# timspilak/cloud_merger

Hardware: NVIDIA B200
Metric: merged+voxel-filtered Mpoints/s (higher is better)
Workload: dtype f32

## Files before the change

### cloud_merger_b200/csrc/cm_api.cu

```cuda
#include <cuda_runtime.h>
#include <dlfcn.h>
#include <sched.h>
#include <nccl.h>

#include <algorithm>
#include <chrono>
#include <cmath>
#include <cstdarg>
#include <cstddef>
#include <cstdio>
#include <cstdlib>
#include <cstring>
#include <limits>
#include <memory>
#include <mutex>
#include <new>
#include <random>
#include <string>
#include <type_traits>
#include <unordered_map>
#include <vector>

#include "../../include/cloud_merger_gpu.h"
#include "cm_kernels.h"
// ... 157 lines not shown
    DevPtr<uint32_t> out_src;
    HostPtr<uint32_t> report;
    cudaStream_t stream = nullptr;
    bool ran = false;
    int64_t launches = 0;
    ZoneParams last{};
    int n_zones_run = 0;
    bool ror_run = false;
  } zw;
  DevPtr<uint32_t> cell_table;
  size_t cell_table_cap = 0;
  DevPtr<float4> stage;
  size_t stage_cap = 0;
  struct SorWs {
    size_t cap = 0;
    DevPtr<float4> sorted_pts;
    DevPtr<float> dist;
    DevPtr<SorStats> stats;
    HostPtr<SorStats> stats_host;
    Event ev[3];
    cudaStream_t stream = nullptr;
    bool ran = false, profiled = false;
    int n_clouds = 0;
    int64_t n_points = 0;
    uint32_t n_valid[CM_MAX_ZONES] = {};
    uint32_t too_few = 0;
  } sw;
  struct PlaneWs {
    size_t cap_draws = 0;
    DevPtr<int32_t> samples_dev;
    DevPtr<int32_t> counts_dev;
    DevPtr<float4> models_dev;
    DevPtr<float> acc_dev;
    HostPtr<int32_t> samples_pin;
    HostPtr<int32_t> counts_pin;
    HostPtr<float4> models_pin;
    HostPtr<float> acc_pin;
  } pw;
  struct ProceedWs {
    size_t cap = 0;
    DevPtr<float4> low, high, rest, planes;
    DevPtr<float4> no_ground, ground;
  } prz;
  std::vector<Slot> slots;
  std::vector<Stream> sensor_stream;
  size_t slot_stride = 0;
  int fill = 0;
  int64_t ticket_counter = 0;
  bool use_graph = true;
  int submit_policy = CM_SUBMIT_LATEST_WINS;
};

namespace {

int fail(cm_handle_t h, int code, const char* fmt, ...) {
  char buf[512];
  va_list ap;
  va_start(ap, fmt);
  vsnprintf(buf, sizeof(buf), fmt, ap);
  va_end(ap);
  if (h) h->last_error = buf;
  return code;
}

#define CM_CUDA(h, expr)                                                                              \
  do {                                                                                                \
    cudaError_t e__ = (expr);                                                                         \
    if (e__ != cudaSuccess) return fail(h, CM_E_CUDA, "%s: %s (%s:%d)", #expr, cudaGetErrorString(e__), \
                                        __FILE__, __LINE__);                                          \
  } while (0)

int numa_node_of_current_device() {
  int dev = 0;
  char bus[64] = {0};
  if (cudaGetDevice(&dev) != cudaSuccess || cudaDeviceGetPCIBusId(bus, (int)sizeof(bus), dev) != cudaSuccess) { cudaGetLastError(); return -1; }
  for (char* c = bus; *c; ++c) *c = (char)tolower(*c);
  char path[160];
  snprintf(path, sizeof(path), "/sys/bus/pci/devices/%s/numa_node", bus);
  FILE* f = fopen(path, "r");
  if (!f) return -1;
  int node = -1;
  if (fscanf(f, "%d", &node) != 1) node = -1;
  fclose(f);
  return node;
}
bool cpus_of_node(int node, cpu_set_t* set) {
  char path[96];
  snprintf(path, sizeof(path), "/sys/devices/system/node/node%d/cpulist", node);
  FILE* f = fopen(path, "r");
  if (!f) return false;
  CPU_ZERO(set);
  int a = 0, b = 0, n = 0;
  char sep = 0;
  while (fscanf(f, "%d", &a) == 1) {
    b = a;
    int c = fgetc(f);
    if (c == '-') { if (fscanf(f, "%d", &b) != 1) break; c = fgetc(f); }
    for (int k = a; k <= b && k < CPU_SETSIZE; ++k) { CPU_SET(k, set); ++n; }
    sep = (char)c;
    if (sep != ',') break;
  }
  fclose(f);
  return n > 0;
}
template <typename T>
cudaError_t pinned_alloc(HostPtr<T>& p, size_t bytes, unsigned flags) {
  static const bool no_numa = getenv("CM_NO_NUMA") != nullptr;
  cpu_set_t old_set, local;
  bool moved = false;
  if (!no_numa) {
    const int node = numa_node_of_current_device();
    if (node >= 0 && cpus_of_node(node, &local) && sched_getaffinity(0, sizeof(old_set), &old_set) == 0) {
      cpu_set_t both;
      CPU_AND(&both, &local, &old_set);
      if (CPU_COUNT(&both) > 0 && !CPU_EQUAL(&both, &old_set)) moved = sched_setaffinity(0, sizeof(both), &both) == 0;
    }
  }
  void* raw = nullptr;
  const cudaError_t e = cudaHostAlloc(&raw, bytes ? bytes : 1, flags);
  if (moved) sched_setaffinity(0, sizeof(old_set), &old_set);
  p.reset(e == cudaSuccess ? static_cast<T*>(raw) : nullptr);
  return e;
}

template <typename T>
cudaError_t dev_alloc(DevPtr<T>& p, size_t count, size_t min_bytes = kAlign) {
  void* raw = nullptr;
  const cudaError_t e = cudaMalloc(&raw, std::max<size_t>(count * sizeof(T), min_bytes));
  p.reset(e == cudaSuccess ? static_cast<T*>(raw) : nullptr);
  return e;
}

template <typename Owner>
cudaError_t create(Owner& p, cudaError_t (*make)(typename Owner::pointer*, unsigned), unsigned flags) {
  typename Owner::pointer raw = nullptr;
  const cudaError_t e = make(&raw, flags);
  p.reset(e == cudaSuccess ? raw : nullptr);
  return e;
}

int ws_alloc(cm_handle_t h, Workspace& w, uint32_t points, uint32_t frames, uint32_t segs, int out_step) {
  w = Workspace();
  w.cap_points = points; w.cap_frames = frames; w.cap_segs = segs; w.out_step = out_step;
  w.ml.build(frames, segs);
  const size_t np = std::max<uint32_t>(points, 1);
  CM_CUDA(h, dev_alloc(w.meta, w.ml.total));
  CM_CUDA(h, cudaMemset(w.meta.get(), 0, w.ml.total));
  CM_CUDA(h, pinned_alloc(w.report, w.ml.total, cudaHostAllocDefault));
  memset(w.report.get(), 0, w.ml.total);
  CM_CUDA(h, dev_alloc(w.segs, segs));
  CM_CUDA(h, dev_alloc(w.surv_xyzi, np));
  CM_CUDA(h, dev_alloc(w.surv_src, np));
  CM_CUDA(h, dev_alloc(w.surv_key, np));
  CM_CUDA(h, dev_alloc(w.first_k1, sort_lookback_rows((uint32_t)np)));
  CM_CUDA(h, dev_alloc(w.keys_a, np, 0));
  CM_CUDA(h, dev_alloc(w.keys_b, np, 0));
  CM_CUDA(h, dev_alloc(w.vals_a, np));
  CM_CUDA(h, dev_alloc(w.vals_b, np));
  w.lb_k1_n = np / k1_min_tile_points() + segs + 2;
  CM_CUDA(h, dev_alloc(w.tile_seg, w.lb_k1_n));
  w.lb_sort_n = (sort_lookback_rows((uint32_t)np) + (frames > 1 ? frames : 0u)) * CM_RADIX;
  if (frames > 1) {
    CM_CUDA(h, dev_alloc(w.seg_tile, sort_lookback_rows((uint32_t)np) + frames));
    CM_CUDA(h, dev_alloc(w.seg_hist, (size_t)frames * CM_SEG_PASSES * CM_RADIX));
    CM_CUDA(h, dev_alloc(w.seg_frame_tile0, (size_t)frames + 1));
    CM_CUDA(h, dev_alloc(w.seg_cent_range, np / centroid_tile_items() + 2));
  }
  w.lb_cent_n = np / centroid_tile_items() + 2;
  CM_CUDA(h, dev_alloc(w.tile_rec, w.lb_k1_n));
  CM_CUDA(h, dev_alloc(w.lb_sort, w.lb_sort_n));
  CM_CUDA(h, dev_alloc(w.cent_status, w.lb_cent_n));
  CM_CUDA(h, cudaMemset(w.cent_status.get(), 0, w.lb_cent_n * 8));
  CM_CUDA(h, cudaMemset(w.lb_sort.get(), 0, w.lb_sort_n * 8));
  CM_CUDA(h, dev_alloc(w.epoch_dev, (size_t)1));
  CM_CUDA(h, cudaMemcpy(w.epoch_dev.get(), &h->epoch_start, sizeof(uint32_t), cudaMemcpyHostToDevice));
  CM_CUDA(h, dev_alloc(w.out_xyzi, np * (size_t)out_step, 0));
  CM_CUDA(h, dev_alloc(w.out_count, np));
  CM_CUDA(h, dev_alloc(w.out_idx, np));
  for (auto& e : w.ev) CM_CUDA(h, create(e, cudaEventCreateWithFlags, cudaEventDefault));
  if (getenv("CM_TRACE")) {
    w.trace_k1_n = w.lb_k1_n * 8; w.trace_sort_n = (w.lb_sort_n / CM_RADIX) * 8;
    CM_CUDA(h, dev_alloc(w.trace_k1, w.trace_k1_n));
    CM_CUDA(h, dev_alloc(w.trace_sort, w.trace_sort_n));
    CM_CUDA(h, cudaMemset(w.trace_k1.get(), 0, w.trace_k1_n * 8));
    CM_CUDA(h, cudaMemset(w.trace_sort.get(), 0, w.trace_sort_n * 8));
  }
  CM_CUDA(h, cudaDeviceSynchronize());
  w.ready = true;
  return CM_OK;
}

uint32_t seg_mode(const cm_layout_t& L) {
  if (L.point_step == 16 && L.off_x == 0 && L.off_y == 4 && L.off_z == 8 && L.off_intensity == 12) return SEG_PACKED16;
  if (L.point_step == 32 && L.off_x == 0 && L.off_y == 4 && L.off_z == 8 && L.off_intensity == 16) return SEG_PCL32;
  const bool a4 = (L.point_step % 4 == 0) && (L.off_x % 4 == 0) && (L.off_y % 4 == 0) && (L.off_z % 4 == 0) &&
                  (L.off_intensity < 0 || L.off_intensity % 4 == 0);
  if (a4) return SEG_ALIGNED4;
  if (L.point_step <= CM_MAX_STAGED_STEP) return SEG_STAGED;
  return SEG_BYTES;
}

bool layout_ok(const cm_layout_t& L) {
  if (L.point_step < 12 || L.point_step > 65535) return false;
  auto in = [&](int off) { return off >= 0 && off + 4 <= L.point_step; };
  if (!in(L.off_x) || !in(L.off_y) || !in(L.off_z)) return false;
  if (L.off_intensity >= 0 && !in(L.off_intensity)) return false;
  return true;
}

inline uint32_t bits_for(unsigned long long count) {
  uint32_t b = 0;
  while (b < 64 && (count - 1ull) >> b) ++b;
  return count <= 1 ? 0 : b;
}

bool crop_cell_bound(cm_handle_t h, unsigned long long* cells) {
  if (h->crop.n_pass <= 0) return false;
  unsigned long long prod = 1;
  for (int a = 0; a < 3; ++a) {
    float lo = -std::numeric_limits<float>::infinity(), hi = std::numeric_limits<float>::infinity();
    for (int k = 0; k < h->crop.n_pass; ++k) {
      const PassDev& ps = h->crop.pass[k];
      if (ps.axis != a || ps.negative) continue;
      if (!(ps.lo == ps.lo) || !(ps.hi == ps.hi)) return false;
      lo = std::max(lo, ps.lo);
      hi = std::min(hi, ps.hi);
    }
    if (!std::isfinite(lo) || !std::isfinite(hi)) return false;
    long long div = 1;
    if (hi >= lo) {
      const float flo = std::floor(lo * h->inv_leaf[a]), fhi = std::floor(hi * h->inv_leaf[a]);
      if (!(std::fabs(flo) < 1e9f) || !(std::fabs(fhi) < 1e9f)) return false;
      div = (long long)fhi - (long long)flo + 1;
    }
    if (div > (1ll << 21)) return false;
    prod *= (unsigned long long)div;
  }
  *cells = prod;
  return true;
}

bool crop_box_grid(cm_handle_t h, uint32_t n_frames, BoxGrid* g) {
  const CropDev& c = h->crop;
  if (!c.is_box) return false;
  const float fmax = std::numeric_limits<float>::max();
  unsigned long long div[3];
  for (int a = 0; a < 3; ++a) {
    if (!(c.lo[a] > -fmax) || !(c.hi[a] < fmax) || !(c.hi[a] >= c.lo[a])) return false;
    const float flo = std::floor(c.lo[a] * h->inv_leaf[a]), fhi = std::floor(c.hi[a] * h->inv_leaf[a]);
    if (!(std::fabs(flo) < 1e9f) || !(std::fabs(fhi) < 1e9f)) return false;
    g->inv[a] = h->inv_leaf[a];
    g->min_b[a] = (int32_t)flo;
    div[a] = (unsigned long long)((long long)fhi - (long long)flo + 1);
    if (div[a] > (1ull << 21)) return false;
  }
  const unsigned long long cells = div[0] * div[1] * div[2];
  const uint32_t idx_bits = bits_for(cells), bits = idx_bits + bits_for(n_frames);
  if (bits > 32u || cells > 0xFFFFFFFFull) return false;
  g->mul1 = (uint32_t)div[0];
  g->mul2 = (uint32_t)(div[0] * div[1]);
  g->idx_bits = idx_bits;
  g->n_pass = std::max<uint32_t>(1u, (bits + CM_RADIX_BITS - 1) / CM_RADIX_BITS);
  return true;
}

void fill_voxel_params(cm_handle_t h, Workspace& w, VoxelParams& vp, const float4* pts, uint32_t n_frames,
                       uint32_t max_points) {
  vp.pts = pts;
  vp.frame_surv_start = reinterpret_cast<uint32_t*>(w.meta.get() + w.ml.off_fstart);
  vp.n_frames = n_frames;
  vp.max_points = max_points;
  for (int k = 0; k < 3; ++k) vp.inv_leaf[k] = h->inv_leaf[k];
  vp.min_points = h->min_points;
  vp.downsample_all = h->downsample_all;
  vp.pcl_refuses = h->overflow_mode == 1 ? 1u : 0u;
  vp.key_bytes = 8;
  vp.out_step = (uint32_t)w.out_step;
  vp.ctrl = reinterpret_cast<Ctrl*>(w.meta.get() + w.ml.off_ctrl);
  vp.acc = reinterpret_cast<FrameAcc*>(w.meta.get() + w.ml.off_acc);
  vp.grid = reinterpret_cast<GridDev*>(w.meta.get() + w.ml.off_grid);
  vp.info = reinterpret_cast<SortInfo*>(w.meta.get() + w.ml.off_info);
  vp.hist = reinterpret_cast<uint32_t*>(w.meta.get() + w.ml.off_hist);
  vp.keys_a = w.keys_a.get(); vp.keys_b = w.keys_b.get(); vp.vals_a = w.vals_a.get(); vp.vals_b = w.vals_b.get();
  vp.lb_sort = w.lb_sort.get(); vp.cent_status = w.cent_status.get();
  vp.cent_status_words = (uint32_t)std::min<size_t>(w.lb_cent_n, 0xFFFFFFFFu);
  vp.tile_rec = w.ran_k1 ? w.tile_rec.get() : nullptr;
  vp.n_k1_tiles = w.n_k1_tiles;
  vp.epoch_dev = w.epoch_dev.get();
  vp.lb_sort_words = (uint32_t)std::min<size_t>(w.lb_sort_n, 0xFFFFFFFFu);
  vp.max_passes = CM_MAX_SORT_PASSES;
  vp.fused_keys = 0; vp.surv_key = w.surv_key.get(); vp.box = BoxGrid{}; vp.first_k1 = w.first_k1.get();
  vp.sort_tile = sort_tile_items(4, max_points);
  vp.dual_width = 0;
  vp.segmented = 0; vp.seg_tile = w.seg_tile.get(); vp.seg_hist = w.seg_hist.get(); vp.seg_frame_tile0 = w.seg_frame_tile0.get();
  vp.seg_cent_range = w.seg_cent_range.get();
  vp.out_xyzi = w.out_xyzi.get(); vp.out_count = w.out_count.get(); vp.out_idx = w.out_idx.get();
  vp.trace = w.trace_sort.get();
  const char* tp = getenv("CM_TRACE_PASS");
  vp.trace_pass = tp ? (uint32_t)atoi(tp) : 1u;
}

int run_voxel(cm_handle_t h, Workspace& w, VoxelParams& vp, cudaStream_t st, bool scan_k1_tiles = false,
              bool with_centroid = true, int known_idx_bits = -1) {
  unsigned long long cells = 0;
  const bool bounded = vp.fused_keys || known_idx_bits >= 0 || (w.ran_k1 && crop_cell_bound(h, &cells));
  if (vp.fused_keys) {
    vp.key_bytes = 4;
    vp.max_passes = vp.box.n_pass;
  } else if (bounded) {
    const uint32_t bits = (known_idx_bits >= 0 ? (uint32_t)known_idx_bits : bits_for(cells)) + bits_for(vp.n_frames);
    vp.key_bytes = bits <= 32 ? 4 : 8;
    vp.max_passes = std::max<uint32_t>(1, (bits + CM_RADIX_BITS - 1) / CM_RADIX_BITS);
  } else {
    vp.key_bytes = 8;
    vp.max_passes = CM_MAX_SORT_PASSES;
  }
  static const bool no_dual = getenv("CM_NO_DUAL") != nullptr;
  const bool dual = !bounded && with_centroid && !no_dual;
  w.dual_width = dual;
  vp.dual_width = dual ? 1u : 0u;
  static const bool no_seg = getenv("CM_NO_SEGMENTED") != nullptr;
  vp.segmented = 0;
  if (!no_seg && with_centroid && vp.n_frames > 1 && w.seg_tile && !vp.fused_keys) {
    if (dual) {
      vp.segmented = 1;
    } else if (bounded) {
      const uint32_t ib = known_idx_bits >= 0 ? (uint32_t)known_idx_bits : bits_for(cells), fb = bits_for(vp.n_frames);
      const uint32_t p_seg = std::max<uint32_t>(1, (ib + CM_RADIX_BITS - 1) / CM_RADIX_BITS);
      if (ib <= 32 && (p_seg < vp.max_passes || ib + fb > 32)) {
        vp.segmented = 2;
        vp.key_bytes = 4;
        vp.max_passes = p_seg;
      }
    }
  }
  w.segmented = vp.segmented != 0;
  if (vp.segmented)
    CM_CUDA(h, cudaMemsetAsync(w.seg_hist.get(), 0, (size_t)vp.n_frames * CM_SEG_PASSES * CM_RADIX * sizeof(uint32_t), st));
  if (scan_k1_tiles)
    CM_CUDA(h, launch_grid_setup(vp, st, w.tile_rec.get(), w.n_k1_tiles, w.segs.get(), w.n_segs,
                                 reinterpret_cast<uint32_t*>(w.meta.get() + w.ml.off_segstart)));
  else
    CM_CUDA(h, launch_grid_setup(vp, st));
  ++w.launches;
  if (h->profiling) CM_CUDA(h, cudaEventRecord(w.ev[EV_GRID].get(), st));
  if (dual) {
    w.key_bytes = 0;
    w.max_passes = CM_MAX_SORT_PASSES;
    VoxelParams v4 = vp, v8 = vp;
    v4.key_bytes = 4; v8.key_bytes = 8;
    CM_CUDA(h, launch_key_hist(v4, st));
    CM_CUDA(h, launch_key_hist(v8, st));
    w.launches += 2;
    if (vp.segmented) {
      CM_CUDA(h, launch_seg_base(v4, st));
      ++w.launches;
    }
    if (h->profiling) CM_CUDA(h, cudaEventRecord(w.ev[EV_KEY].get(), st));
    for (uint32_t ps = 0; ps < 4; ++ps) CM_CUDA(h, launch_sort_pass(v4, (int)ps, st));
    for (uint32_t ps = 0; ps < CM_MAX_SORT_PASSES; ++ps) CM_CUDA(h, launch_sort_pass(v8, (int)ps, st));
    w.launches += 4 + CM_MAX_SORT_PASSES;
    if (h->profiling) CM_CUDA(h, cudaEventRecord(w.ev[EV_SORT].get(), st));
    CM_CUDA(h, launch_centroid(v4, st));
    CM_CUDA(h, launch_centroid(v8, st));
    w.launches += 2 * CM_CENTROID_LAUNCHES;
    if (!w.capturing) CM_CUDA(h, cudaEventRecord(w.ev[EV_CENT].get(), st));
    w.ran_voxel = true;
    return CM_OK;
  }
  if (!bounded) {
    SortInfo si;
    Ctrl ctrl;
    CM_CUDA(h, cudaMemcpyAsync(w.report.get(), w.meta.get(), w.ml.off_info + sizeof(SortInfo), cudaMemcpyDeviceToHost, st));
    CM_CUDA(h, cudaStreamSynchronize(st));
    memcpy(&si, w.report.get() + w.ml.off_info, sizeof(si));
    memcpy(&ctrl, w.report.get() + w.ml.off_ctrl, sizeof(ctrl));
    vp.key_bytes = si.total_bits <= 32 ? 4 : 8;
    vp.max_passes = si.num_passes;
    w.plan_idx_bits = si.idx_bits; w.plan_total_bits = si.total_bits; w.plan_error = ctrl.error;
  }
  w.key_bytes = vp.key_bytes;
  w.max_passes = vp.max_passes;
  if (!vp.fused_keys) {
    CM_CUDA(h, launch_key_hist(vp, st));
    ++w.launches;
  }
  if (vp.segmented) {
    CM_CUDA(h, launch_seg_base(vp, st));
    ++w.launches;
  }
  if (h->profiling) CM_CUDA(h, cudaEventRecord(w.ev[EV_KEY].get(), st));
  w.timed_pass0 = false;
  for (uint32_t ps = 0; ps < vp.max_passes; ++ps) {
    CM_CUDA(h, launch_sort_pass(vp, (int)ps, st));
    ++w.launches;
    if (ps == 0 && h->profiling) {
      CM_CUDA(h, cudaEventRecord(w.ev[EV_SORT0].get(), st));
      w.timed_pass0 = true;
    }
  }
  if (h->profiling) CM_CUDA(h, cudaEventRecord(w.ev[EV_SORT].get(), st));
  if (!with_centroid) {
    w.ran_voxel = false;
    return CM_OK;
  }
  CM_CUDA(h, launch_centroid(vp, st));
  w.launches += CM_CENTROID_LAUNCHES;
  if (!w.capturing) CM_CUDA(h, cudaEventRecord(w.ev[EV_CENT].get(), st));
  w.ran_voxel = true;
  return CM_OK;
}

template <typename Chain>
void derive_box(Chain& c) {
  const float fmax = std::numeric_limits<float>::max();
  c.is_box = 0; c.use_i = 0;
  for (int a = 0; a < 4; ++a) { c.lo[a] = -fmax; c.hi[a] = fmax; }
  if (c.n_pass <= 0) return;
  for (int k = 0; k < c.n_pass; ++k) {
    const PassDev& ps = c.pass[k];
    if (ps.negative || !(ps.lo == ps.lo) || !(ps.hi == ps.hi)) return;
    c.lo[ps.axis] = std::max(c.lo[ps.axis], ps.lo);
    c.hi[ps.axis] = std::min(c.hi[ps.axis], ps.hi);
    if (ps.axis == 3) c.use_i = 1;
  }
  c.is_box = 1;
}

struct SegPlan {
  uint32_t n_frames = 0, n_tiles = 0, tile_points = 0, tiles_per_seg = 0, staged_smem = 0;
  int mode = -1;
  int64_t total_points = 0;
};

int build_segments(cm_handle_t h, Workspace& w, const cm_segment_t* segs, int n_seg, std::vector<SegDev>& out,
                   std::vector<uint32_t>& tile_seg, SegPlan* plan) {
  if (n_seg <= 0 || !segs) return fail(h, CM_E_INVALID, "no segments");
  if ((uint32_t)n_seg > w.cap_segs) return fail(h, CM_E_CAPACITY, "%d segments > capacity %u", n_seg, w.cap_segs);
  int64_t total = 0;
  uint32_t max_step_staged = 0;
  int common_mode = -2;
  for (int s = 0; s < n_seg; ++s) {
    const cm_segment_t& g = segs[s];
    if (!layout_ok(g.layout)) return fail(h, CM_E_INVALID, "segment %d: bad layout", s);
    if (g.n_points < 0 || g.n_points > 0xFFFFFFF0ll) return fail(h, CM_E_INVALID, "segment %d: bad n_points", s);
    if (g.n_points > 0 && (!g.data || (reinterpret_cast<uintptr_t>(g.data) & 15u)))
      return fail(h, CM_E_INVALID, "segment %d: data must be a 16-byte aligned device pointer", s);
    if (g.sensor < 0 || g.sensor >= h->cfg.max_sensors) return fail(h, CM_E_INVALID, "segment %d: bad sensor", s);
    if (s == 0 ? g.frame != 0 : (g.frame != segs[s - 1].frame && g.frame != segs[s - 1].frame + 1))
      return fail(h, CM_E_INVALID, "segment %d: frames must start at 0 and increase by steps of 1", s);
    const int md = (int)seg_mode(g.layout);
    if (md == (int)SEG_STAGED) max_step_staged = std::max<uint32_t>(max_step_staged, (uint32_t)g.layout.point_step);
    common_mode = (common_mode == -2 || common_mode == md) ? md : -1;
    total += g.n_points;
  }
  if (total > (int64_t)w.cap_points) return fail(h, CM_E_CAPACITY, "%lld points > capacity %u", (long long)total, w.cap_points);
  uint32_t T = k1_tile_points(total);
  if (max_step_staged && k1_staged_smem(T, max_step_staged) > 200u * 1024u) T = k1_min_tile_points();
  out.resize(n_seg);
  uint32_t tile = 0, frame = 0, src_base = 0;
  uint64_t slot_base = 0;
  bool uniform = true;
  uint32_t tps = 0;
  for (int s = 0; s < n_seg; ++s) {
    const cm_segment_t& g = segs[s];
    const bool first = (s == 0) || (g.frame != segs[s - 1].frame);
    if (first) { frame = (uint32_t)g.frame; src_base = 0; }
    SegDev& d = out[s];
    memset(&d, 0, sizeof(d));
    d.data = static_cast<const uint8_t*>(g.data);
    d.n_points = (uint32_t)g.n_points;
    d.tile_begin = tile;
    d.src_base = src_base;
    d.slot_base = (uint32_t)slot_base;
    d.frame = frame;
    d.point_step = g.layout.point_step;
    d.off_x = g.layout.off_x; d.off_y = g.layout.off_y; d.off_z = g.layout.off_z;
    d.off_i = g.layout.off_intensity >= 0 ? g.layout.off_intensity : -1;
    d.is_dense = g.layout.is_dense ? 1u : 0u;
    d.sensor = (uint32_t)g.sensor;
    d.first_of_frame = first ? 1u : 0u;
    d.mode = seg_mode(g.layout);
    memcpy(d.m, h->mats_host + g.sensor * 12, sizeof(d.m));
    const uint32_t nt = std::max<uint32_t>(1u, (d.n_points + T - 1) / T);
    if (s == 0) tps = nt; else if (nt != tps) uniform = false;
    tile += nt;
    src_base += d.n_points;
    slot_base += d.n_points;
  }
  if (frame + 1 > w.cap_frames) return fail(h, CM_E_CAPACITY, "%u frames > capacity %u", frame + 1, w.cap_frames);
  if ((size_t)tile + 1 > w.lb_k1_n) return fail(h, CM_E_CAPACITY, "too many tiles");
  if (slot_base > 0xFFFFFFF0ull) return fail(h, CM_E_CAPACITY, "batch too large");
  tile_seg.clear();
  if (!uniform) {
    tile_seg.resize(tile);
    for (int s = 0; s < n_seg; ++s) {
      const uint32_t te = (s + 1 < n_seg) ? out[s + 1].tile_begin : tile;
      for (uint32_t t = out[s].tile_begin; t < te; ++t) tile_seg[t] = (uint32_t)s;
    }
  }
  plan->n_frames = frame + 1; plan->n_tiles = tile; plan->tile_points = T; plan->total_points = total;
  plan->tiles_per_seg = uniform ? tps : 0u;
  plan->mode = (common_mode == (int)SEG_PACKED16 || common_mode == (int)SEG_PCL32) ? common_mode : -1;
  plan->staged_smem = max_step_staged ? k1_staged_smem(T, max_step_staged) : 0u;
  return CM_OK;
}

int run_pipeline(cm_handle_t h, Workspace& w, const cm_segment_t* segs, int n_seg, cudaStream_t st, bool with_voxel) {
  SegPlan plan;
  std::vector<SegDev> sd;
  std::vector<uint32_t> ts;
  int rc = build_segments(h, w, segs, n_seg, sd, ts, &plan);
  if (rc != CM_OK) return rc;
  if (sd.size() != w.segs_host.size() || memcmp(sd.data(), w.segs_host.data(), sd.size() * sizeof(SegDev)) != 0) {
    CM_CUDA(h, cudaMemcpyAsync(w.segs.get(), sd.data(), sd.size() * sizeof(SegDev), cudaMemcpyHostToDevice, st));
    w.segs_host = sd;
  }
  if (!ts.empty() && ts != w.tile_seg_host) {
    CM_CUDA(h, cudaMemcpyAsync(w.tile_seg.get(), ts.data(), ts.size() * sizeof(uint32_t), cudaMemcpyHostToDevice, st));
    w.tile_seg_host = ts;
  }
  const uint32_t n_frames = plan.n_frames;
  const int64_t total = plan.total_points;
  w.has_run = true; w.report_valid = false; w.profiled = h->profiling;
  w.n_frames = n_frames; w.n_segs = (uint32_t)n_seg; w.points_in = total; w.launches = 0;
  w.ran_k1 = true; w.ran_voxel = false; w.stream = st;
  w.voxel_pts = w.surv_xyzi.get();
  h->last = &w; h->zone_launches = false;

  if (!w.capturing) CM_CUDA(h, cudaEventRecord(w.ev[EV_START].get(), st));
  CM_CUDA(h, cudaMemsetAsync(w.meta.get(), 0, w.ml.zero_bytes, st));
  K1Params kp;
  kp.segs = w.segs.get(); kp.n_seg = (uint32_t)n_seg; kp.n_tiles = plan.n_tiles; kp.n_frames = n_frames;
  kp.tiles_per_seg = plan.tiles_per_seg; kp.tile_seg = w.tile_seg.get();
  kp.crop = h->crop;
  kp.surv_xyzi = w.surv_xyzi.get(); kp.surv_src = w.surv_src.get();
  kp.ctrl = reinterpret_cast<Ctrl*>(w.meta.get() + w.ml.off_ctrl);
  kp.acc = reinterpret_cast<FrameAcc*>(w.meta.get() + w.ml.off_acc);
  kp.tile_rec = w.tile_rec.get();
  kp.trace = w.trace_k1.get();
  static const bool no_fused = getenv("CM_NO_FUSED_KEYS") != nullptr;
  BoxGrid box{};
  const bool fused = with_voxel && !no_fused && crop_box_grid(h, n_frames, &box);
  w.fused_keys = fused; w.box = box;
  kp.surv_key = fused ? w.surv_key.get() : nullptr;
  kp.hist = reinterpret_cast<uint32_t*>(w.meta.get() + w.ml.off_hist);
  kp.box = box;
  kp.obox = nullptr; kp.n_obox = 0;
  if (h->n_obox > 0) {
    const std::vector<OrientedBoxDev> ob(h->obox, h->obox + h->n_obox);
    if (!w.obox) CM_CUDA(h, dev_alloc(w.obox, CM_MAX_CROP_BOXES));
    if (ob.size() != w.obox_host.size() || memcmp(ob.data(), w.obox_host.data(), ob.size() * sizeof(OrientedBoxDev)) != 0) {
      CM_CUDA(h, cudaMemcpyAsync(w.obox.get(), ob.data(), ob.size() * sizeof(OrientedBoxDev), cudaMemcpyHostToDevice, st));
      w.obox_host = ob;
    }
    kp.obox = w.obox.get(); kp.n_obox = (uint32_t)h->n_obox;
  }
  w.n_k1_tiles = plan.n_tiles;
  w.dense_valid = false;
  CM_CUDA(h, launch_transform_crop(kp, plan.tile_points, plan.mode, plan.staged_smem, st));
  ++w.launches;
  if (!with_voxel) {
    CM_CUDA(h, launch_tile_scan(w.tile_rec.get(), plan.n_tiles, w.segs.get(), (uint32_t)n_seg, n_frames,
                                reinterpret_cast<uint32_t*>(w.meta.get() + w.ml.off_fstart),
                                reinterpret_cast<uint32_t*>(w.meta.get() + w.ml.off_segstart), st));
    ++w.launches;
    CM_CUDA(h, cudaEventRecord(w.ev[EV_K1].get(), st));
    return CM_OK;
  }
  if (!w.capturing) CM_CUDA(h, cudaEventRecord(w.ev[EV_K1].get(), st));
  VoxelParams vp;
  fill_voxel_params(h, w, vp, w.surv_xyzi.get(), n_frames, (uint32_t)total);
  vp.fused_keys = fused ? 1u : 0u;
  vp.box = box;
  return run_voxel(h, w, vp, st, true);
}

int materialize_dense(cm_handle_t h, Workspace& w) {
  if (!w.ran_k1 || w.dense_valid) return CM_OK;
  const size_t np = std::max<uint32_t>(w.cap_points, 1);
  if (!w.dense_xyzi) {
    DevPtr<float4> xyzi; DevPtr<uint32_t> src, slot;
    CM_CUDA(h, dev_alloc(xyzi, np));
    CM_CUDA(h, dev_alloc(src, np));
    CM_CUDA(h, dev_alloc(slot, np));
    w.dense_xyzi = std::move(xyzi); w.dense_src = std::move(src); w.dense_slot = std::move(slot);
  }
  CM_CUDA(h, launch_compact_survivors(w.tile_rec.get(), w.n_k1_tiles, w.surv_xyzi.get(), w.surv_src.get(), w.dense_xyzi.get(),
                                      w.dense_src.get(), w.dense_slot.get(), w.stream));
  w.dense_valid = true;
  return CM_OK;
}

int fetch_report(cm_handle_t h, Workspace& w, cudaEvent_t already_copied = nullptr) {
  if (!w.has_run) return fail(h, CM_E_INVALID, "nothing has run on this handle");
  if (w.report_valid) return CM_OK;
  if (already_copied) {
    CM_CUDA(h, cudaEventSynchronize(already_copied));
  } else {
    CM_CUDA(h, cudaMemcpyAsync(w.report.get(), w.meta.get(), w.ml.total, cudaMemcpyDeviceToHost, w.stream));
    CM_CUDA(h, cudaStreamSynchronize(w.stream));
  }
  const Ctrl* ctrl = reinterpret_cast<const Ctrl*>(w.report.get() + w.ml.off_ctrl);
  const FrameAcc* acc = reinterpret_cast<const FrameAcc*>(w.report.get() + w.ml.off_acc);
  const SortInfo* si = reinterpret_cast<const SortInfo*>(w.report.get() + w.ml.off_info);
  const uint32_t* fstart = reinterpret_cast<const uint32_t*>(w.report.get() + w.ml.off_fstart);
  const GridDev* grid = reinterpret_cast<const GridDev*>(w.report.get() + w.ml.off_grid);
  cm_stats_t& s = h->stats;
  memset(&s, 0, sizeof(s));
  s.points_in = w.points_in;
  s.frames = (int32_t)w.n_frames;
  s.survivors = fstart[w.n_frames];
  s.device_error = (int32_t)ctrl->error;
  h->frame_info.assign(w.n_frames, cm_frame_info_t{});
  int64_t vbeg = 0;
  for (uint32_t f = 0; f < w.n_frames; ++f) {
    cm_frame_info_t& fi = h->frame_info[f];
    fi.survivor_begin = fstart[f];
    fi.survivor_end = fstart[f + 1];
    if (w.ran_voxel) {
      fi.voxel_begin = vbeg;
      vbeg += acc[f].voxel_count;
      fi.voxel_end = vbeg;
      for (int k = 0; k < 3; ++k) { fi.min_b[k] = grid[f].min_b[k]; fi.max_b[k] = grid[f].max_b[k]; fi.div_b[k] = grid[f].div_b[k]; }
      fi.pcl_overflow = grid[f].pcl_overflow;
      s.pcl_overflow += grid[f].pcl_overflow;
    }
  }
  if (w.ran_voxel) {
    s.voxels_out = ctrl->total_voxels;
    s.key_bits = (int32_t)si->total_bits;
    s.sort_passes = (int32_t)si->num_passes;
    if (w.dual_width) w.key_bytes = si->width == 4u ? 4u : 8u;
    s.key_bytes = (int32_t)w.key_bytes;
  }
  const int last_ev = w.ran_voxel ? EV_CENT : EV_K1;
  float ms = 0.f;
  if (cudaEventElapsedTime(&ms, w.ev[EV_START].get(), w.ev[last_ev].get()) == cudaSuccess) s.gpu_ms = ms;
  else cudaGetLastError();
  for (auto& v : h->stage_ms) v = -1.f;
  h->stage_ms[EV_START] = s.gpu_ms;
  if (w.profiled) {
    float t;
    if (cudaEventElapsedTime(&t, w.ev[EV_START].get(), w.ev[EV_K1].get()) == cudaSuccess) h->stage_ms[EV_K1] = t;
    if (w.ran_voxel) {
      if (cudaEventElapsedTime(&t, w.ev[EV_K1].get(), w.ev[EV_GRID].get()) == cudaSuccess) h->stage_ms[EV_GRID] = t;
      if (cudaEventElapsedTime(&t, w.ev[EV_GRID].get(), w.ev[EV_KEY].get()) == cudaSuccess) h->stage_ms[EV_KEY] = t;
      if (cudaEventElapsedTime(&t, w.ev[EV_KEY].get(), w.ev[EV_SORT].get()) == cudaSuccess) h->stage_ms[EV_SORT] = t;
      if (w.timed_pass0 && cudaEventElapsedTime(&t, w.ev[EV_KEY].get(), w.ev[EV_SORT0].get()) == cudaSuccess) h->stage_ms[EV_SORT0] = t;
      if (cudaEventElapsedTime(&t, w.ev[EV_SORT].get(), w.ev[EV_CENT].get()) == cudaSuccess) h->stage_ms[EV_CENT] = t;
    }
  }
  w.report_valid = true;
  if (ctrl->error == CM_DEV_E_KEY_RANGE) return fail(h, CM_E_KEY_RANGE, "voxel grid exceeds the key range (leaf too small for the extent)");
  if (ctrl->error) return fail(h, CM_E_INTERNAL, "device watchdog tripped (code %u)", ctrl->error);
  return CM_OK;
}

int ensure_batch_ws(cm_handle_t h) {
  if (h->batch.ready) return CM_OK;
  const cm_config_t& c = h->cfg;
  return ws_alloc(h, h->batch, (uint32_t)c.max_batch_points, (uint32_t)c.max_batch_frames, (uint32_t)c.max_batch_segments,
                  c.out_point_step);
}

int ensure_host_path(cm_handle_t h) {
  if (!h->slots.empty()) return CM_OK;
  const cm_config_t& c = h->cfg;
  h->slot_stride = align_up((size_t)c.max_points_per_sensor * (size_t)c.max_point_step + 16, kAlign);
  std::vector<Stream> streams(c.max_sensors);
  for (auto& s : streams) CM_CUDA(h, create(s, cudaStreamCreateWithFlags, cudaStreamNonBlocking));
  std::vector<Slot> slots(c.frames_in_flight);
  const uint64_t pts = (uint64_t)c.max_sensors * (uint64_t)c.max_points_per_sensor;
  if (pts > 0xFFFFFFF0ull) return fail(h, CM_E_CAPACITY, "max_sensors * max_points_per_sensor too large");
  for (auto& sl : slots) {
    int rc = ws_alloc(h, sl.ws, (uint32_t)pts, 1, (uint32_t)c.max_sensors, c.out_point_step);
    if (rc != CM_OK) return rc;
    CM_CUDA(h, dev_alloc(sl.raw_dev, h->slot_stride * c.max_sensors, 0));
    CM_CUDA(h, pinned_alloc(sl.raw_pinned, h->slot_stride * c.max_sensors, cudaHostAllocDefault));
    sl.arena_bytes = 2 * h->slot_stride * c.max_sensors;
    CM_CUDA(h, dev_alloc(sl.arena_dev, sl.arena_bytes, 0));
    sl.exp_cap = (uint32_t)pts;
    const size_t ecap = std::max<size_t>(sl.exp_cap, 1);
    CM_CUDA(h, pinned_alloc(sl.exp_xyzi, ecap * (size_t)c.out_point_step, cudaHostAllocMapped));
    CM_CUDA(h, pinned_alloc(sl.exp_count, ecap * sizeof(uint32_t), cudaHostAllocMapped));
    CM_CUDA(h, pinned_alloc(sl.exp_idx, ecap * sizeof(unsigned long long), cudaHostAllocMapped));
    sl.sensor.resize(c.max_sensors);
    for (auto& ss : sl.sensor) CM_CUDA(h, create(ss.copied, cudaEventCreateWithFlags, cudaEventDisableTiming));
    CM_CUDA(h, create(sl.stream, cudaStreamCreateWithFlags, cudaStreamNonBlocking));
    CM_CUDA(h, create(sl.done, cudaEventCreateWithFlags, cudaEventDisableTiming));
  }
  h->sensor_stream = std::move(streams);
  h->slots = std::move(slots);
  return CM_OK;
}

int submit_impl(cm_handle_t h, int sensor, const void* data, int64_t n_points, const cm_layout_t* layout, uint64_t stamp,
                bool pinned_src) {
  if (!h) return CM_E_INVALID;
// ... 2301 lines not shown
```

### cloud_merger_b200/csrc/cm_common.cuh

```cuda
#pragma once

#include <cuda_runtime.h>
#include <stdint.h>

#define CM_RADIX_BITS 8
#define CM_RADIX 256
#define CM_MAX_SORT_PASSES 8

#define CM_DEV_OK 0
#define CM_DEV_E_KEY_RANGE 5
#define CM_DEV_E_INTERNAL 6

namespace cm {

enum SegMode : uint32_t {
  SEG_PACKED16 = 0,
  SEG_PCL32 = 1,
  SEG_ALIGNED4 = 2,
  SEG_STAGED = 3,
  SEG_BYTES = 4
};
#define CM_MAX_STAGED_STEP 96

struct SegDev {
  const uint8_t* data;
  uint32_t n_points;
  uint32_t tile_begin;
  uint32_t src_base;
  uint32_t slot_base;
  uint32_t frame;
  int32_t point_step;
  int32_t off_x, off_y, off_z, off_i;
  uint32_t is_dense;
  uint32_t sensor;
  uint32_t first_of_frame;
  uint32_t mode;
  uint32_t pad_;
  float m[12];
  uint32_t pad2_[3];
};
static_assert(sizeof(SegDev) == 128, "SegDev must stay 128 bytes");

struct PassDev {
  int32_t axis;
  float lo, hi;
  int32_t negative;
};

struct CropDev {
  int32_t n_pass;
  PassDev pass[8];
  int32_t is_box;
  int32_t use_i;
  float lo[4], hi[4];
};

#define CM_MAX_CROP_BOXES 8
#define OBOX_TRANSFORM 1u
#define OBOX_TRANSLATE 2u
#define OBOX_ROTATE 4u
#define OBOX_NEGATIVE 8u
struct OrientedBoxDev {
  float t[12];
  float r[12];
  float tr[3];
  float mn[3], mx[3];
  uint32_t flags;
  uint32_t pad_[2];
};
static_assert(sizeof(OrientedBoxDev) == 144, "OrientedBoxDev is loaded as 16-byte words");

#define CM_MAX_ZONES 16
#define CM_MAX_ZONE_PASSES 4
struct ZoneDev {
  int32_t n_pass;
  PassDev pass[CM_MAX_ZONE_PASSES];
  int32_t is_box, use_i;
  float lo[4], hi[4];
};
struct ZoneSet {
  int32_t n_zones;
  int32_t all_box;
  ZoneDev zone[CM_MAX_ZONES];
};

struct TileRec {
  uint32_t count;
  uint32_t slot0;
  uint32_t frame;
  uint32_t dense0;
};

struct FrameAcc {
  uint32_t max_enc[3];
  uint32_t nmin_enc[3];
  uint32_t n_invalid;
  uint32_t voxel_count;
};

struct Ctrl {
  uint32_t tile_counter[12];
  uint32_t error;
  uint32_t total_voxels;
  uint32_t has_invalid;
  uint32_t pad_;
  uint32_t role_counter[CM_MAX_SORT_PASSES];
  uint32_t cent_ticket;
  uint32_t pad2_[7];
};
static_assert(sizeof(Ctrl) == 128, "Ctrl is two cache lines");

struct GridDev {
  int32_t min_b[3];
  int32_t max_b[3];
  int32_t div_b[3];
  int32_t pcl_overflow;
  uint32_t bits;
  uint32_t empty;
  uint32_t zero_keys;
  unsigned long long mul1, mul2;
};

struct SortInfo {
  uint32_t num_passes;
  uint32_t total_bits;
  uint32_t idx_bits;
  uint32_t n_keys;
  uint32_t key_frames;
  uint32_t width;
  uint32_t segmented;
  uint32_t n_seg_tiles;
};

struct SegTile {
  uint32_t base;
  uint32_t n;
  uint32_t frame;
  uint32_t pad;
};
constexpr uint32_t CM_SEG_FIRST = 0x80000000u;
constexpr uint32_t CM_SEG_PASSES = 4;

__host__ __device__ __forceinline__ uint32_t f32_order_enc(uint32_t bits) {
  return bits ^ ((bits >> 31) ? 0xFFFFFFFFu : 0x80000000u);
}
__host__ __device__ __forceinline__ uint32_t f32_order_dec(uint32_t enc) {
  return enc ^ ((enc >> 31) ? 0x80000000u : 0xFFFFFFFFu);
}

#ifdef __CUDACC__

__device__ __forceinline__ bool finite_f32(float v) { return (__float_as_uint(v) & 0x7F800000u) != 0x7F800000u; }

__device__ __forceinline__ uint32_t lane_id() { return threadIdx.x & 31u; }
__device__ __forceinline__ uint32_t lanemask_lt() {
  uint32_t m;
  asm("mov.u32 %0, %%lanemask_lt;" : "=r"(m));
  return m;
}

__device__ __forceinline__ uint32_t warp_sum_u32(uint32_t v) {
#pragma unroll
  for (int o = 16; o > 0; o >>= 1) v += __shfl_xor_sync(0xFFFFFFFFu, v, o);
  return v;
}
__device__ __forceinline__ uint32_t warp_incl_scan_u32(uint32_t v) {
  const uint32_t lane = lane_id();
#pragma unroll
  for (int o = 1; o < 32; o <<= 1) {
    uint32_t t = __shfl_up_sync(0xFFFFFFFFu, v, o);
    if (lane >= (uint32_t)o) v += t;
  }
  return v;
}

__device__ __forceinline__ float4 ldg_stream_f4(const void* p) {
  float4 r;
  asm volatile("ld.global.nc.L1::no_allocate.v4.f32 {%0,%1,%2,%3}, [%4];"
               : "=f"(r.x), "=f"(r.y), "=f"(r.z), "=f"(r.w)
               : "l"(p));
  return r;
}
__device__ __forceinline__ float ldg_stream_f1(const void* p) {
  float r;
  asm volatile("ld.global.nc.L1::no_allocate.f32 %0, [%1];" : "=f"(r) : "l"(p));
  return r;
}

#define CM_LB_AGG 1u
#define CM_LB_INCL 2u
#define CM_SPIN_LIMIT (1u << 22)
#define CM_WATCHDOG_NS 4000000000ull
#define CM_WATCHDOG_STRIDE 1024u

__device__ __forceinline__ unsigned long long lb_pack(uint32_t epoch, uint32_t flag, uint32_t value) {
  return ((unsigned long long)(epoch * 4u + flag) << 32) | (unsigned long long)value;
}

__device__ __forceinline__ unsigned long long ld_relaxed_u64(const unsigned long long* p) {
  unsigned long long v;
  asm volatile("ld.relaxed.gpu.global.u64 %0, [%1];" : "=l"(v) : "l"(p) : "memory");
  return v;
}
__device__ __forceinline__ unsigned long long ld_cg_u64(const unsigned long long* p) {
  unsigned long long v;
  asm volatile("ld.global.cg.u64 %0, [%1];" : "=l"(v) : "l"(p));
  return v;
}
__device__ __forceinline__ void st_cg_u64(unsigned long long* p, unsigned long long v) {
  asm volatile("st.global.cg.u64 [%0], %1;" ::"l"(p), "l"(v) : "memory");
}
__device__ __forceinline__ void st_relaxed_u64(unsigned long long* p, unsigned long long v) {
  asm volatile("st.relaxed.gpu.global.u64 [%0], %1;" ::"l"(p), "l"(v) : "memory");
}

__device__ __forceinline__ bool lb_ready(unsigned long long w, uint32_t epoch) {
  const uint32_t hi = (uint32_t)(w >> 32);
  return (hi >> 2) == epoch && (hi & 3u) != 0u;
}

__device__ __forceinline__ unsigned long long global_timer_ns() {
  unsigned long long t;
  asm volatile("mov.u64 %0, %%globaltimer;" : "=l"(t));
  return t;
}
__device__ __forceinline__ bool watchdog_expired(uint32_t& spins, unsigned long long& t0) {
  if ((++spins & (CM_WATCHDOG_STRIDE - 1u)) != 0u) return false;
  const unsigned long long now = global_timer_ns();
  if (t0 == 0ull) {
    t0 = now;
    return false;
  }
  return now - t0 > CM_WATCHDOG_NS;
}

__device__ __forceinline__ uint32_t lb_wait_inclusive(unsigned long long* p, uint32_t epoch, uint32_t* err) {
  uint32_t spins = 0;
  unsigned long long t0 = 0ull;
  while (true) {
    const unsigned long long w = ld_relaxed_u64(p);
    const uint32_t hi = (uint32_t)(w >> 32);
    if ((hi >> 2) == epoch && (hi & 3u) == CM_LB_INCL) return (uint32_t)w;
    if (watchdog_expired(spins, t0)) {
      atomicExch(err, (uint32_t)CM_DEV_E_INTERNAL);
      return 0u;
    }
    if (spins > 16) __nanosleep(40);
  }
}

__device__ __forceinline__ uint32_t block_excl_scan_256(uint32_t v, uint32_t* scratch, uint32_t* total) {
  const uint32_t tid = threadIdx.x, lane = tid & 31u, w = tid >> 5;
  if (tid >= 256) v = 0;
  const uint32_t incl = warp_incl_scan_u32(v);
  if (lane == 31 && w < 8) scratch[w] = incl;
  __syncthreads();
  if (tid == 0) {
    uint32_t run = 0;
#pragma unroll
    for (int i = 0; i < 8; ++i) {
      uint32_t t = scratch[i];
      scratch[i] = run;
      run += t;
    }
    scratch[8] = run;
  }
  __syncthreads();
  const uint32_t res = incl - v + (w < 8 ? scratch[w] : 0u);
  *total = scratch[8];
  __syncthreads();
  return res;
}

#endif

}
```

### cloud_merger_b200/csrc/cm_kernels.h

```cpp
#pragma once

#include <algorithm>

#include "cm_common.cuh"

namespace cm {

#define K1_BIG_BATCH_POINTS (1u << 21)
struct BoxGrid {
  float inv[3];
  int32_t min_b[3];
  uint32_t mul1, mul2;
  uint32_t idx_bits;
  uint32_t n_pass;
};
struct K1Params {
  const SegDev* segs;
  uint32_t n_seg;
  uint32_t n_tiles;
  uint32_t n_frames;
  uint32_t tiles_per_seg;
  const uint32_t* tile_seg;
  CropDev crop;
  float4* surv_xyzi;
  uint32_t* surv_src;
  Ctrl* ctrl;
  FrameAcc* acc;
  uint32_t* surv_key;
  uint32_t* hist;
  BoxGrid box;
  TileRec* tile_rec;
  unsigned long long* trace;
  const OrientedBoxDev* obox;
  uint32_t n_obox;
};
uint32_t k1_tile_points(int64_t total_points);
uint32_t k1_min_tile_points();
uint32_t k1_staged_smem(uint32_t tile_points, uint32_t max_step);
cudaError_t launch_transform_crop(const K1Params& p, uint32_t tile_points, int mode, uint32_t staged_smem_bytes,
                                  cudaStream_t stream);

cudaError_t launch_tile_scan(TileRec* tile_rec, uint32_t n_tiles, const SegDev* segs, uint32_t n_seg, uint32_t n_frames,
                             uint32_t* frame_surv_start, uint32_t* seg_surv_start, cudaStream_t stream);
cudaError_t launch_compact_survivors(const TileRec* tile_rec, uint32_t n_tiles, const float4* slot_xyzi,
                                     const uint32_t* slot_src, float4* dense_xyzi, uint32_t* dense_src,
                                     uint32_t* dense_slot, cudaStream_t stream);

struct VoxelParams {
  const float4* pts;
  const TileRec* tile_rec;
  uint32_t n_k1_tiles;
  const uint32_t* frame_surv_start;
  uint32_t n_frames;
  uint32_t max_points;
  float inv_leaf[3];
  uint32_t min_points;
  uint32_t downsample_all;
  uint32_t pcl_refuses;
  uint32_t key_bytes;
  uint32_t out_step;
  Ctrl* ctrl;
  FrameAcc* acc;
  GridDev* grid;
  SortInfo* info;
  uint32_t* hist;
  void* keys_a;
  void* keys_b;
  uint32_t* vals_a;
  uint32_t* vals_b;
  unsigned long long* lb_sort;
  unsigned long long* cent_status;
  uint32_t cent_status_words;
  uint32_t* epoch_dev;
  uint32_t lb_sort_words;
  uint32_t max_passes;
  uint32_t fused_keys;
  const uint32_t* surv_key;
  BoxGrid box;
  uint32_t* first_k1;
  uint32_t sort_tile;
  uint32_t dual_width;
  uint32_t segmented;
  SegTile* seg_tile;
  uint32_t* seg_hist;
  uint32_t* seg_frame_tile0;
  uint2* seg_cent_range;
  void* out_xyzi;
  uint32_t* out_count;
  unsigned long long* out_idx;
  unsigned long long* trace;
  uint32_t trace_pass;
};

cudaError_t launch_minmax(const float4* pts, uint32_t n, Ctrl* ctrl, FrameAcc* acc, uint32_t* frame_surv_start,
                          cudaStream_t stream);
cudaError_t launch_seed_bounds(FrameAcc* acc, const float* mn, const float* mx, cudaStream_t stream);
cudaError_t launch_grid_setup(const VoxelParams& p, cudaStream_t stream, TileRec* scan_rec = nullptr, uint32_t scan_tiles = 0,
                              const SegDev* segs = nullptr, uint32_t n_seg = 0, uint32_t* seg_surv_start = nullptr);
cudaError_t launch_key_hist(const VoxelParams& p, cudaStream_t stream);
cudaError_t launch_seg_base(const VoxelParams& p, cudaStream_t stream);
cudaError_t launch_seg_keys64(const void* records, unsigned long long* keys, uint32_t* vals, const VoxelParams& p,
                              cudaStream_t stream);
cudaError_t launch_sort_pass(const VoxelParams& p, int pass, cudaStream_t stream);
cudaError_t launch_split_records(const void* records, uint32_t* keys, uint32_t* vals, const uint32_t* n_ptr,
                                 uint32_t max_points, cudaStream_t stream, const VoxelParams* remap = nullptr);
cudaError_t launch_centroid(const VoxelParams& p, cudaStream_t stream);
#define CM_CENTROID_LAUNCHES 1
cudaError_t launch_export_voxels(const VoxelParams& p, void* host_xyzi, uint32_t* host_count, unsigned long long* host_idx,
                                 uint32_t cap, cudaStream_t stream);

struct GiantPlan;
struct ZoneParams {
  const float4* pts;
  uint32_t n_points;
  uint32_t n_tiles;
  ZoneSet zones;
  unsigned short* mask;
  uint32_t mask_given;
  uint32_t* tile_count;
  uint32_t* tile_offset;
  uint32_t* zone_total;
  uint32_t* scan_ticket;
  uint32_t* zone_begin;
  uint32_t* overflow;
  uint32_t out_capacity;
  float4* out_xyzi;
  uint32_t* out_src;
  float4* zone_ptr[CM_MAX_ZONES];
  const uint32_t* zone_remote_base;
  const GiantPlan* giant_plan;
  uint32_t giant_invalid_part;
};
struct RorParams {
  float r2;
  uint32_t min_pts;
  uint32_t negative;
  unsigned short* mask;
  uint32_t* cell_start;
  uint32_t table_keys;
};
cudaError_t launch_radius_table(const VoxelParams& p, const RorParams& r, cudaStream_t stream);
cudaError_t launch_radius_count(const VoxelParams& p, const RorParams& r, cudaStream_t stream);

struct SorParams {
  uint32_t mean_k;
  uint32_t sqrt_mode;
  uint32_t too_few;
  const float4* sorted_pts;
  float* dist;
  const uint32_t* cell_start;
  double cell;
};
struct SorStats {
  double sum, sq_sum, mean, stddev, threshold;
  uint32_t path;
  uint32_t pad_;
};
struct SorSumParams {
  const float* dist;
  uint32_t n_clouds;
  uint32_t begin[CM_MAX_ZONES + 1];
  uint32_t n_valid[CM_MAX_ZONES];
  uint32_t too_few;
  uint32_t force_serial;
  uint32_t negative;
  double std_mul;
  SorStats* stats;
  unsigned short* mask;
};
cudaError_t launch_sor_knn(const VoxelParams& p, const SorParams& s, float4* sorted_pts, cudaStream_t stream);
cudaError_t launch_sor_sums(const SorSumParams& s, cudaStream_t stream);
cudaError_t launch_sor_select(const SorSumParams& s, uint32_t n_points, cudaStream_t stream);

#define CM_MAX_PLANE_CLOUDS (CM_MAX_ZONES / 2)
struct PlaneParams {
  const float4* pts;
  uint32_t n_clouds;
  uint32_t begin[CM_MAX_PLANE_CLOUDS + 1];
  uint32_t n_draws[CM_MAX_PLANE_CLOUDS];
  uint32_t draw_stride;
  float threshold;
  uint32_t sum_order;
// ... 79 lines not shown
```

### cloud_merger_b200/csrc/cm_radix_sort.cu

```cuda
#include <cstdio>
#include <cstdlib>

#include "cm_kernels.h"

namespace cm {

namespace {

#ifndef RS_THREADS_CFG
#define RS_THREADS_CFG 384
#endif
#ifndef RS_IPT32
#define RS_IPT32 12
#endif
#ifndef RS_IPT64
#define RS_IPT64 8
#endif
#ifndef RS_MIN_CTAS
#define RS_MIN_CTAS 2
#endif
#ifndef RS_EARLY_COUNT
#define RS_EARLY_COUNT 0
#endif
constexpr int RS_THREADS = RS_THREADS_CFG;
static_assert(RS_THREADS >= CM_RADIX && RS_THREADS % 32 == 0, "one thread per digit is needed");
constexpr int RS_WARPS = RS_THREADS / 32;

template <typename KeyT>
struct SortCfg;
template <>
struct SortCfg<uint32_t> {
  static constexpr int IPT = RS_IPT32;
};
template <>
struct SortCfg<unsigned long long> {
  static constexpr int IPT = RS_IPT64;
};

constexpr int RS_SCANNERS = 8;
constexpr int RS_SCAN_DIGITS = CM_RADIX / RS_SCANNERS;
constexpr int RS_SCAN_ROWS = 32;
constexpr int RS_SCAN_GROUP = RS_THREADS >= 512 ? 8 : 16;
static_assert(RS_SCAN_DIGITS == 32, "one digit per lane");

template <bool SEG>
__device__ __forceinline__ void scanner_cta(uint32_t scanner , unsigned long long* rows ,
                                            uint32_t n_tiles, uint32_t epoch, const uint32_t* hist ,
                                            uint32_t* err, uint32_t* s_scan, uint32_t* s_tmp ,
                                            unsigned long long* s_chain , const SegTile* __restrict__ seg_tile,
                                            const uint32_t* __restrict__ seg_base ) {
  const uint32_t tid = threadIdx.x, lane = tid & 31u, q = tid >> 5;
  const uint32_t d = scanner * RS_SCAN_DIGITS + lane;
  if (SEG) {
    if (q == 0) s_chain[lane] = 0ull;
  } else {
    uint32_t tot;
    const uint32_t gb = block_excl_scan_256(tid < CM_RADIX ? hist[tid] : 0u, s_scan, &tot);
    if (tid < CM_RADIX) s_tmp[tid] = gb;
    __syncthreads();
    if (q == 0) {
      const uint32_t run0 = s_tmp[d];
      st_cg_u64(rows - CM_RADIX + d, lb_pack(epoch, CM_LB_INCL, run0));
      s_chain[lane] = (unsigned long long)run0;
    }
  }
  __syncthreads();
  const uint32_t n_batches = (n_tiles + RS_SCAN_ROWS - 1) / RS_SCAN_ROWS;
  volatile unsigned long long* chain = s_chain + lane;
  for (uint32_t b = q; b < n_batches; b += RS_WARPS) {
    const uint32_t r0 = b * RS_SCAN_ROWS;
    unsigned long long* const base = rows + (size_t)r0 * CM_RADIX + d;
    uint32_t c[RS_SCAN_ROWS];
#pragma unroll
    for (int g0 = 0; g0 < RS_SCAN_ROWS; g0 += RS_SCAN_GROUP) {
      uint32_t spins = 0;
      unsigned long long wd0 = 0ull;
      while (true) {
        unsigned long long w[RS_SCAN_GROUP];
#pragma unroll
        for (int k = 0; k < RS_SCAN_GROUP; ++k)
          w[k] = (r0 + g0 + k < n_tiles) ? ld_cg_u64(base + (size_t)(g0 + k) * CM_RADIX) : lb_pack(epoch, CM_LB_AGG, 0u);
        bool all = true;
#pragma unroll
        for (int k = 0; k < RS_SCAN_GROUP; ++k) {
          all = all && lb_ready(w[k], epoch);
          c[g0 + k] = (uint32_t)w[k];
        }
        if (__all_sync(0xFFFFFFFFu, all)) break;
        if (__any_sync(0xFFFFFFFFu, watchdog_expired(spins, wd0))) {
          atomicExch(err, (uint32_t)CM_DEV_E_INTERNAL);
          break;
        }
        if (spins > 8) __nanosleep(50);
      }
    }
    uint32_t sum = 0;
    uint32_t abs_from = RS_SCAN_ROWS;
    if (SEG) {
      const uint32_t mine = (r0 + lane < n_tiles) ? __ldg(&seg_tile[r0 + lane].frame) : 0u;
      const uint32_t firsts = __ballot_sync(0xFFFFFFFFu, (mine & CM_SEG_FIRST) != 0u);
      if (firsts) abs_from = (uint32_t)__ffs(firsts) - 1u;
#pragma unroll
      for (int k = 0; k < RS_SCAN_ROWS; ++k) {
        if (firsts & (1u << k)) {
          const uint32_t f = __shfl_sync(0xFFFFFFFFu, mine, k) & ~CM_SEG_FIRST;
          sum = __ldg(seg_base + (size_t)f * (CM_SEG_PASSES * CM_RADIX) + d);
        }
        sum += c[k];
        c[k] = sum;
      }
    } else {
#pragma unroll
      for (int k = 0; k < RS_SCAN_ROWS; ++k) {
        sum += c[k];
        c[k] = sum;
      }
    }
    unsigned long long x = *chain;
    uint32_t spins = 0;
    unsigned long long wd0 = 0ull;
    while ((uint32_t)(x >> 32) != b) {
      if (watchdog_expired(spins, wd0)) {
        atomicExch(err, (uint32_t)CM_DEV_E_INTERNAL);
        break;
      }
      x = *chain;
    }
    const uint32_t run = (uint32_t)x;
    if (SEG) {
      *chain = ((unsigned long long)(b + 1u) << 32) | (unsigned long long)(abs_from < RS_SCAN_ROWS ? sum : run + sum);
#pragma unroll
      for (int k = 0; k < RS_SCAN_ROWS; ++k)
        if (r0 + k < n_tiles)
          st_cg_u64(base + (size_t)k * CM_RADIX, lb_pack(epoch, CM_LB_INCL, (uint32_t)k >= abs_from ? c[k] : run + c[k]));
    } else {
      *chain = ((unsigned long long)(b + 1u) << 32) | (unsigned long long)(run + sum);
#pragma unroll
      for (int k = 0; k < RS_SCAN_ROWS; ++k)
        if (r0 + k < n_tiles) st_cg_u64(base + (size_t)k * CM_RADIX, lb_pack(epoch, CM_LB_INCL, run + c[k]));
    }
  }
}

__device__ __forceinline__ uint32_t warp_diff8(uint32_t x) {
  uint32_t t[8];
#pragma unroll
  for (int b = 0; b < 8; ++b) {
    asm volatile(
        "{\n .reg .pred p;\n .reg .b32 y;\n and.b32 y, %1, %2;\n setp.ne.u32 p, y, 0;\n"
        " vote.sync.ballot.b32 %0, p, 0xffffffff;\n @p not.b32 %0, %0;\n}"
        : "=r"(t[b])
        : "r"(x), "r"(1u << b));
  }
  uint32_t a, c;
  asm("lop3.b32 %0, %1, %2, %3, 0xFE;" : "=r"(a) : "r"(t[0]), "r"(t[1]), "r"(t[2]));
  asm("lop3.b32 %0, %1, %2, %3, 0xFE;" : "=r"(c) : "r"(t[3]), "r"(t[4]), "r"(t[5]));
  asm("lop3.b32 %0, %1, %2, %3, 0xFE;" : "=r"(a) : "r"(a), "r"(t[6]), "r"(t[7]));
  return a | c;
}

__device__ __forceinline__ uint32_t lanemask_gt() {
  uint32_t m;
  asm("mov.u32 %0, %%lanemask_gt;" : "=r"(m));
  return m;
}

template <typename KeyT, int IPT>
struct SortSmem {
  static constexpr int TILE = RS_THREADS * IPT;
  static constexpr bool AOS = sizeof(KeyT) == 4;
  unsigned long long k[2][TILE];
  uint32_t v[2][AOS ? 1 : TILE];
  uint32_t hist[RS_WARPS * CM_RADIX];
  uint32_t scatter[2][CM_RADIX];
  uint32_t scan[12];
  uint32_t cnt[CM_RADIX];
  uint32_t later[3][CM_RADIX];
  uint32_t next_tile[2];
};

template <typename KeyT, int IPT, bool FUSED0 = false, bool SEG = false>
__global__ void __launch_bounds__(RS_THREADS, RS_MIN_CTAS) k_onesweep_pass(const VoxelParams p, const int pass) {
  static_assert(!SEG || (sizeof(KeyT) == 4 && !FUSED0), "segmented keys are 32-bit records written by k_voxel_key_hist");
  constexpr int TILE = RS_THREADS * IPT;
  constexpr int WARP_ITEMS = 32 * IPT;
  constexpr bool AOS = sizeof(KeyT) == 4;
  extern __shared__ __align__(16) unsigned char s_raw[];
  SortSmem<KeyT, IPT>& sm = *reinterpret_cast<SortSmem<KeyT, IPT>*>(s_raw);

  const long long tr0 = clock64();
  const SortInfo si = *p.info;
  if ((uint32_t)pass >= si.num_passes) return;
  if (p.dual_width && ((si.width == 4u) != (sizeof(KeyT) == 4))) return;
  if (SEG != (si.segmented != 0u)) return;
  const uint32_t M = si.n_keys;
  const uint32_t n_tiles = SEG ? si.n_seg_tiles : (M + TILE - 1) / TILE;
  const uint32_t* const seg_base = SEG ? p.seg_hist + (size_t)pass * CM_RADIX : nullptr;

  const uint32_t tid = threadIdx.x, lane = tid & 31u;
  const uint32_t warp = __shfl_sync(0xFFFFFFFFu, tid >> 5, 0);
  const uint32_t epoch = *p.epoch_dev + 1u + (uint32_t)pass;
  unsigned long long* const rows = p.lb_sort + CM_RADIX;
  uint32_t* const err = &p.ctrl->error;
  uint32_t* const counter = &p.ctrl->tile_counter[1 + pass];
  if (tid == 0) {
    const uint32_t role = atomicAdd(&p.ctrl->role_counter[pass], 1u);
    sm.next_tile[1] = role;
    if (role >= (uint32_t)RS_SCANNERS) sm.next_tile[0] = atomicAdd(counter, 1u);
  }
  __syncthreads();
  const uint32_t role = sm.next_tile[1];
  if (role < (uint32_t)RS_SCANNERS) {
    __syncthreads();
    scanner_cta<SEG>(role, rows, n_tiles, epoch, p.hist + pass * CM_RADIX, err, sm.scan, sm.hist, &sm.k[0][0], p.seg_tile, seg_base);
    return;
  }

#define RS_TRACE(t, i, t0) do { if (p.trace && p.trace_pass == (uint32_t)pass && tid == 0) p.trace[(size_t)(t) * 8 + (i)] = (unsigned long long)(clock64() - (t0)); } while (0)
  const bool odd = (pass & 1) != 0;
  const uint32_t shift = (uint32_t)pass * CM_RADIX_BITS;
  const uint32_t lt = lanemask_lt(), gt = lanemask_gt();
  uint32_t* const wh = sm.hist + warp * CM_RADIX;

  if (RS_EARLY_COUNT && tid < CM_RADIX) sm.cnt[tid] = 0;
  if (FUSED0)
    for (uint32_t i = tid; i < 3u * CM_RADIX; i += RS_THREADS) (&sm.later[0][0])[i] = 0u;
  uint32_t cur = sm.next_tile[0];
  __syncthreads();
  uint32_t prev = 0xFFFFFFFFu, prev_n = 0;
  uint32_t prev_seg = 0;
  uint32_t buf = 0;
  long long tr_cur = tr0, tr_prev = tr0;
  uint32_t claimed = 0xFFFFFFFFu;
  while (true) {
    tr_prev = tr_cur;
    tr_cur = clock64();
    const bool have = cur < n_tiles;
    uint32_t n_here = 0;
    uint32_t cur_seg = 0;
    if (have) {
      uint32_t tile_base = cur * TILE;
      if (SEG) {
        const uint4 q = __ldg(reinterpret_cast<const uint4*>(p.seg_tile + cur));
        tile_base = q.x; n_here = q.y; cur_seg = q.z;
      } else {
        n_here = min((uint32_t)TILE, M - tile_base);
      }
      const bool full = n_here == (uint32_t)TILE;
      const uint32_t item0 = warp * WARP_ITEMS + lane;
      KeyT key[IPT];
      uint32_t val[IPT];
      if (FUSED0) {
        const uint32_t k1_first = p.first_k1[cur];
        const uint32_t e = k1_first + lane;
        uint32_t e_dense = 0xFFFFFFFFu, e_slot = 0u, e_end = 0xFFFFFFFFu;
        if (e < p.n_k1_tiles) {
          const uint4 q = __ldg(reinterpret_cast<const uint4*>(p.tile_rec + e));
          e_dense = q.w; e_slot = q.y; e_end = q.w + q.x;
        }
        const uint32_t last_end = __shfl_sync(0xFFFFFFFFu, e_end, 31);
        const bool covered = last_end >= tile_base + n_here;
        const uint32_t w0 = tile_base + warp * WARP_ITEMS;
        uint32_t kk = (uint32_t)__popc(__ballot_sync(0xFFFFFFFFu, e_dense <= w0));
        kk = kk ? kk - 1u : 0u;
        const uint32_t* __restrict__ tdense = reinterpret_cast<const uint32_t*>(p.tile_rec);
#pragma unroll
        for (int i = 0; i < IPT; ++i) {
          const uint32_t d = tile_base + item0 + 32 * i;
          uint32_t slot;
          if (covered) {
            bool adv;
            do {
              const uint32_t nd = __shfl_sync(0xFFFFFFFFu, e_dense, (kk + 1u) & 31u);
              adv = kk < 31u && nd <= d;
              kk += adv ? 1u : 0u;
            } while (__any_sync(0xFFFFFFFFu, adv));
            slot = __shfl_sync(0xFFFFFFFFu, e_slot, kk) + (d - __shfl_sync(0xFFFFFFFFu, e_dense, kk));
          } else {
            uint32_t lo = k1_first, hi = p.n_k1_tiles - 1u;
            while (lo < hi) {
              const uint32_t mid = (lo + hi + 1u) >> 1;
              if (tdense[mid * 4u + 3u] <= d) lo = mid; else hi = mid - 1u;
            }
            slot = tdense[lo * 4u + 1u] + (d - tdense[lo * 4u + 3u]);
          }
          const bool in = d < M;
          key[i] = in ? (KeyT)p.surv_key[slot] : ~(KeyT)0;
          val[i] = in ? slot : 0u;
        }
#pragma unroll
        for (int i = 0; i < IPT; ++i) {
          if (tile_base + item0 + 32 * i < M) {
#pragma unroll
            for (uint32_t ps = 1; ps < 4; ++ps)
              if (ps < si.num_passes) atomicAdd(&sm.later[ps - 1][((uint32_t)key[i] >> (ps * CM_RADIX_BITS)) & (CM_RADIX - 1)], 1u);
          }
        }
      } else if (AOS) {
        const uint2* __restrict__ in = reinterpret_cast<const uint2*>(odd ? p.keys_b : p.keys_a) + tile_base + item0;
        if (full) {
#pragma unroll
          for (int i = 0; i < IPT; ++i) {
            const uint2 r = in[32 * i];
            key[i] = (KeyT)r.x;
            val[i] = r.y;
          }
        } else {
#pragma unroll
          for (int i = 0; i < IPT; ++i) {
            uint2 r = make_uint2(0xFFFFFFFFu, 0u);
            if (item0 + 32 * i < n_here) r = in[32 * i];
            key[i] = (KeyT)r.x;
            val[i] = r.y;
          }
        }
      } else {
        const KeyT* __restrict__ in_keys = reinterpret_cast<const KeyT*>(odd ? p.keys_b : p.keys_a) + tile_base + item0;
        const uint32_t* __restrict__ in_vals = (odd ? p.vals_b : p.vals_a) + tile_base + item0;
        if (full) {
#pragma unroll
          for (int i = 0; i < IPT; ++i) key[i] = in_keys[32 * i];
#pragma unroll
          for (int i = 0; i < IPT; ++i) val[i] = in_vals[32 * i];
        } else {
#pragma unroll
          for (int i = 0; i < IPT; ++i) key[i] = (item0 + 32 * i < n_here) ? in_keys[32 * i] : ~(KeyT)0;
#pragma unroll
          for (int i = 0; i < IPT; ++i) val[i] = (item0 + 32 * i < n_here) ? in_vals[32 * i] : 0u;
        }
      }
#pragma unroll
      for (int k = 0; k < CM_RADIX / 32; ++k) wh[lane + 32 * k] = 0;
      __syncwarp();
      RS_TRACE(cur, 0, tr_cur);
      if (RS_EARLY_COUNT) {
#pragma unroll
        for (int i = 0; i < IPT; ++i) atomicAdd(&sm.cnt[(uint32_t)(key[i] >> shift) & (CM_RADIX - 1)], 1u);
        __syncthreads();
        if (RS_THREADS == CM_RADIX || tid < CM_RADIX) {
          const uint32_t c = sm.cnt[tid];
          sm.cnt[tid] = 0;
          const uint32_t real = (tid == CM_RADIX - 1) ? c - ((uint32_t)TILE - n_here) : c;
          st_relaxed_u64(rows + (size_t)cur * CM_RADIX + tid, lb_pack(epoch, CM_LB_AGG, real));
        }
      }

      uint32_t rank[IPT];
#pragma unroll
      for (int i = 0; i < IPT; ++i) {
        const uint32_t ks = (uint32_t)(key[i] >> shift);
        const uint32_t diff = warp_diff8(ks);
        const uint32_t below = (uint32_t)__popc(~diff & lt);
        volatile uint32_t* c = wh + (ks & (CM_RADIX - 1));
        const uint32_t r = *c + below;
        rank[i] = r;
        if ((~diff & gt) == 0u) *c = r + 1u;
        __syncwarp();
      }
      __syncthreads();
      RS_TRACE(cur, 1, tr_cur);

      {
        const bool dt = RS_THREADS == CM_RADIX || tid < CM_RADIX;
        uint32_t wc[RS_WARPS];
        uint32_t cnt = 0;
        if (dt) {
#pragma unroll
          for (int w = 0; w < RS_WARPS; ++w) {
            wc[w] = sm.hist[w * CM_RADIX + tid];
            cnt += wc[w];
          }
          if (!RS_EARLY_COUNT) {
            const uint32_t real = (tid == CM_RADIX - 1) ? cnt - ((uint32_t)TILE - n_here) : cnt;
            st_relaxed_u64(rows + (size_t)cur * CM_RADIX + tid, lb_pack(epoch, CM_LB_AGG, real));
          }
        }
        RS_TRACE(cur, 2, tr_cur);
        uint32_t tot;
        const uint32_t bin_start = block_excl_scan_256(cnt, sm.scan, &tot);
        if (dt) {
          uint32_t run = bin_start;
#pragma unroll
          for (int w = 0; w < RS_WARPS; ++w) {
            sm.hist[w * CM_RADIX + tid] = run;
            run += wc[w];
          }
          sm.scatter[buf][tid] = 0u - bin_start;
        }
      }
      __syncthreads();
      RS_TRACE(cur, 3, tr_cur);

#pragma unroll
      for (int i = 0; i < IPT; ++i) {
        const uint32_t ks = (uint32_t)(key[i] >> shift);
        const uint32_t pos = wh[ks & (CM_RADIX - 1)] + rank[i];
        if (AOS) {
          sm.k[buf][pos] = ((unsigned long long)val[i] << 32) | (unsigned long long)key[i];
        } else {
          sm.k[buf][pos] = (unsigned long long)key[i];
          sm.v[buf][pos] = val[i];
        }
      }
      RS_TRACE(cur, 4, tr_cur);
    }
    if (prev != 0xFFFFFFFFu) {
      const uint32_t pb = buf ^ 1u;
      RS_TRACE(prev, 7, tr_prev);
      if (RS_THREADS == CM_RADIX || tid < CM_RADIX) {
        uint32_t first;
        if (SEG && (prev_seg & CM_SEG_FIRST))
          first = __ldg(seg_base + (size_t)(prev_seg & ~CM_SEG_FIRST) * (CM_SEG_PASSES * CM_RADIX) + tid);
        else
          first = lb_wait_inclusive(rows + ((long long)prev - 1) * CM_RADIX + tid, epoch, err);
        sm.scatter[pb][tid] += first;
      }
      __syncthreads();
      RS_TRACE(prev, 5, tr_prev);
      if (tid == 0 && have) claimed = atomicAdd(counter, 1u);
      const bool pfull = prev_n == (uint32_t)TILE;
      const unsigned long long* sk = sm.k[pb];
      const uint32_t* ssc = sm.scatter[pb];
      if (AOS) {
        unsigned long long* __restrict__ out = reinterpret_cast<unsigned long long*>(odd ? p.keys_a : p.keys_b);
        if (pfull) {
          unsigned long long r[IPT];
#pragma unroll
          for (int j = 0; j < IPT; ++j) r[j] = sk[j * RS_THREADS + tid];
#pragma unroll
          for (int j = 0; j < IPT; ++j) {
            const uint32_t dg = ((uint32_t)r[j] >> shift) & (CM_RADIX - 1);
            out[ssc[dg] + (j * RS_THREADS + tid)] = r[j];
          }
        } else {
          for (uint32_t pos = tid; pos < prev_n; pos += RS_THREADS) {
            const unsigned long long r = sk[pos];
            const uint32_t dg = ((uint32_t)r >> shift) & (CM_RADIX - 1);
            out[ssc[dg] + pos] = r;
          }
        }
      } else {
        KeyT* __restrict__ out_keys = reinterpret_cast<KeyT*>(odd ? p.keys_a : p.keys_b);
        uint32_t* __restrict__ out_vals = odd ? p.vals_a : p.vals_b;
        const uint32_t* sv = sm.v[pb];
        if (pfull) {
#pragma unroll
          for (int j0 = 0; j0 < IPT; j0 += 4) {
            unsigned long long kk[4];
            uint32_t vv[4];
#pragma unroll
            for (int j = 0; j < 4 && j0 + j < IPT; ++j) {
              kk[j] = sk[(j0 + j) * RS_THREADS + tid];
              vv[j] = sv[(j0 + j) * RS_THREADS + tid];
            }
#pragma unroll
            for (int j = 0; j < 4 && j0 + j < IPT; ++j) {
              const uint32_t dg = (uint32_t)(kk[j] >> shift) & (CM_RADIX - 1);
              const uint32_t dst = ssc[dg] + ((j0 + j) * RS_THREADS + tid);
              out_keys[dst] = (KeyT)kk[j];
              out_vals[dst] = vv[j];
            }
          }
        } else {
          for (uint32_t pos = tid; pos < prev_n; pos += RS_THREADS) {
            const unsigned long long kk = sk[pos];
            const uint32_t dg = (uint32_t)(kk >> shift) & (CM_RADIX - 1);
            const uint32_t dst = ssc[dg] + pos;
            out_keys[dst] = (KeyT)kk;
            out_vals[dst] = sv[pos];
          }
        }
      }
      RS_TRACE(prev, 6, tr_prev);
    } else if (tid == 0 && have) {
      claimed = atomicAdd(counter, 1u);
    }
    if (!have) break;
    if (tid == 0) sm.next_tile[buf ^ 1u] = claimed;
    prev = cur;
    prev_n = n_here;
    prev_seg = cur_seg;
    buf ^= 1u;
    __syncthreads();
    cur = sm.next_tile[buf];
  }
  if (FUSED0) {
    __syncthreads();
    for (uint32_t i = tid; i < 3u * CM_RADIX; i += RS_THREADS) {
      const uint32_t c = (&sm.later[0][0])[i];
      if (c && (i >> 8) + 1u < si.num_passes) atomicAdd(p.hist + CM_RADIX + i, c);
    }
  }
}

__global__ void __launch_bounds__(256) k_split_records(const uint2* __restrict__ rec, uint32_t* __restrict__ keys,
                                                       uint32_t* __restrict__ vals, const uint32_t* n_ptr, const BoxGrid box,
                                                       const GridDev* __restrict__ grid, const SortInfo* info, uint32_t n_frames) {
  const uint32_t n = *n_ptr;
  const uint32_t idx_bits = info ? info->idx_bits : 0u;
  for (uint32_t i = blockIdx.x * 256u + threadIdx.x; i < n; i += gridDim.x * 256u) {
    const uint2 r = rec[i];
    uint32_t key = r.x;
    if (grid) {
      const uint32_t f = idx_bits < 32u ? key >> idx_bits : 0u;
      const uint32_t b = idx_bits < 32u ? key & ((1u << idx_bits) - 1u) : key;
      const uint32_t k2 = b / box.mul2, r2 = b - k2 * box.mul2, k1 = r2 / box.mul1, k0 = r2 - k1 * box.mul1;
      const GridDev* g = grid + (f < n_frames ? f : 0u);
      const long long c0 = (long long)k0 + box.min_b[0] - g->min_b[0], c1 = (long long)k1 + box.min_b[1] - g->min_b[1],
                      c2 = (long long)k2 + box.min_b[2] - g->min_b[2];
      key = (idx_bits < 32u ? f << idx_bits : 0u) | (uint32_t)(c0 + c1 * (long long)g->mul1 + c2 * (long long)g->mul2);
    }
    keys[i] = key;
    vals[i] = r.y;
  }
}

}

constexpr int RS_IPT_SMALL = 4;
constexpr uint32_t RS_SMALL_LIMIT = 148u * 2u * RS_THREADS * RS_IPT32;

static bool sort_uses_small_tile(uint32_t max_points) { return max_points <= RS_SMALL_LIMIT; }

uint32_t sort_tile_items(uint32_t key_bytes, uint32_t max_points) {
  if (sort_uses_small_tile(max_points)) return RS_THREADS * RS_IPT_SMALL;
  return key_bytes == 4 ? RS_THREADS * SortCfg<uint32_t>::IPT : RS_THREADS * SortCfg<unsigned long long>::IPT;
}

size_t sort_lookback_rows(uint32_t capacity) {
  const uint32_t small_part = std::min(capacity, RS_SMALL_LIMIT);
  const size_t rows_small = small_part / (RS_THREADS * RS_IPT_SMALL) + 1;
  const size_t rows_big = capacity / (RS_THREADS * std::min<int>(SortCfg<uint32_t>::IPT, SortCfg<unsigned long long>::IPT)) + 1;
  return std::max(rows_small, rows_big) + 2;
}

namespace {
template <typename KeyT, int IPT, bool FUSED0 = false, bool SEG = false>
struct PassLaunch {
  static inline int ctas_per_sm = 0;
  static cudaError_t configure() {
    cudaError_t e = cudaFuncSetAttribute(k_onesweep_pass<KeyT, IPT, FUSED0, SEG>, cudaFuncAttributeMaxDynamicSharedMemorySize,
                                         (int)sizeof(SortSmem<KeyT, IPT>));
    if (e != cudaSuccess) return e;
    return cudaOccupancyMaxActiveBlocksPerMultiprocessor(&ctas_per_sm, k_onesweep_pass<KeyT, IPT, FUSED0, SEG>, RS_THREADS,
                                                         sizeof(SortSmem<KeyT, IPT>));
  }
  static cudaError_t launch(const VoxelParams& p, int pass, int sms, cudaStream_t stream) {
    const uint32_t tile = RS_THREADS * IPT;
    const uint32_t tiles = (p.max_points + tile - 1) / tile + (SEG ? p.n_frames : 0u);
    if (tiles == 0) return cudaSuccess;
    const uint32_t workers = std::min<uint32_t>(tiles, (uint32_t)(sms * std::max(1, ctas_per_sm)) - RS_SCANNERS);
    k_onesweep_pass<KeyT, IPT, FUSED0, SEG><<<workers + RS_SCANNERS, RS_THREADS, sizeof(SortSmem<KeyT, IPT>), stream>>>(p, pass);
    return cudaGetLastError();
  }
};
bool g_sort_configured = false;
}

cudaError_t configure_sort_kernels() {
  if (g_sort_configured) return cudaSuccess;
  cudaError_t e = PassLaunch<uint32_t, SortCfg<uint32_t>::IPT>::configure();
  if (e == cudaSuccess) e = PassLaunch<unsigned long long, SortCfg<unsigned long long>::IPT>::configure();
  if (e == cudaSuccess) e = PassLaunch<uint32_t, RS_IPT_SMALL>::configure();
  if (e == cudaSuccess) e = PassLaunch<unsigned long long, RS_IPT_SMALL>::configure();
  if (e == cudaSuccess) e = PassLaunch<uint32_t, SortCfg<uint32_t>::IPT, true>::configure();
  if (e == cudaSuccess) e = PassLaunch<uint32_t, RS_IPT_SMALL, true>::configure();
  if (e == cudaSuccess) e = PassLaunch<uint32_t, SortCfg<uint32_t>::IPT, false, true>::configure();
  if (e == cudaSuccess) e = PassLaunch<uint32_t, RS_IPT_SMALL, false, true>::configure();
  if (e != cudaSuccess) return e;
  if (getenv("CM_DEBUG"))
    fprintf(stderr, "[cm] sort pass CTAs per SM: %d / %d (32 / 64-bit keys), small tile %d / %d\n",
            PassLaunch<uint32_t, SortCfg<uint32_t>::IPT>::ctas_per_sm,
            PassLaunch<unsigned long long, SortCfg<unsigned long long>::IPT>::ctas_per_sm,
            PassLaunch<uint32_t, RS_IPT_SMALL>::ctas_per_sm, PassLaunch<unsigned long long, RS_IPT_SMALL>::ctas_per_sm);
  g_sort_configured = true;
  return cudaSuccess;
}

cudaError_t launch_sort_pass(const VoxelParams& p, int pass, cudaStream_t stream) {
  int dev = 0, sms = 148;
  cudaGetDevice(&dev);
  cudaDeviceGetAttribute(&sms, cudaDevAttrMultiProcessorCount, dev);
  const bool small = sort_uses_small_tile(p.max_points);
  if (p.fused_keys && pass == 0)
    return small ? PassLaunch<uint32_t, RS_IPT_SMALL, true>::launch(p, pass, sms, stream)
                 : PassLaunch<uint32_t, SortCfg<uint32_t>::IPT, true>::launch(p, pass, sms, stream);
  if (p.key_bytes == 4 && p.segmented)
    return small ? PassLaunch<uint32_t, RS_IPT_SMALL, false, true>::launch(p, pass, sms, stream)
                 : PassLaunch<uint32_t, SortCfg<uint32_t>::IPT, false, true>::launch(p, pass, sms, stream);
  if (p.key_bytes == 4)
    return small ? PassLaunch<uint32_t, RS_IPT_SMALL>::launch(p, pass, sms, stream)
                 : PassLaunch<uint32_t, SortCfg<uint32_t>::IPT>::launch(p, pass, sms, stream);
  return small ? PassLaunch<unsigned long long, RS_IPT_SMALL>::launch(p, pass, sms, stream)
               : PassLaunch<unsigned long long, SortCfg<unsigned long long>::IPT>::launch(p, pass, sms, stream);
}

cudaError_t launch_split_records(const void* records, uint32_t* keys, uint32_t* vals, const uint32_t* n_ptr,
                                 uint32_t max_points, cudaStream_t stream, const VoxelParams* remap) {
  if (max_points == 0) return cudaSuccess;
  const uint32_t blocks = std::min<uint32_t>((max_points + 255u) / 256u, 148u * 8u);
  k_split_records<<<blocks, 256, 0, stream>>>(reinterpret_cast<const uint2*>(records), keys, vals, n_ptr,
                                              remap ? remap->box : BoxGrid{}, remap ? remap->grid : nullptr,
                                              remap ? remap->info : nullptr, remap ? remap->n_frames : 0u);
  return cudaGetLastError();
}

}
```

### cloud_merger_b200/csrc/cm_transform_crop.cu

```cuda
#include <cstdlib>

#include "cm_kernels.h"

namespace cm {

namespace {

constexpr int MODE_GENERIC = -1;

__device__ __forceinline__ uint32_t smem_u32(const void* p) { return (uint32_t)__cvta_generic_to_shared(p); }

__device__ __forceinline__ void mbar_init(unsigned long long* bar, uint32_t count) {
  asm volatile("mbarrier.init.shared::cta.b64 [%0], %1;" ::"r"(smem_u32(bar)), "r"(count) : "memory");
  asm volatile("fence.mbarrier_init.release.cluster;" ::: "memory");
}
__device__ __forceinline__ void mbar_arrive_expect_tx(unsigned long long* bar, uint32_t bytes) {
  asm volatile("mbarrier.arrive.expect_tx.shared::cta.b64 _, [%0], %1;" ::"r"(smem_u32(bar)), "r"(bytes) : "memory");
}
__device__ __forceinline__ void bulk_g2s(void* dst_smem, const void* src_gmem, uint32_t bytes, unsigned long long* bar) {
  asm volatile("cp.async.bulk.shared::cluster.global.mbarrier::complete_tx::bytes [%0], [%1], %2, [%3];" ::"r"(
                   smem_u32(dst_smem)),
               "l"(src_gmem), "r"(bytes), "r"(smem_u32(bar))
               : "memory");
}
// ... 196 lines not shown
          y[i] = lds_f32_unaligned(stage, r + oy);
          z[i] = lds_f32_unaligned(stage, r + oz);
          if (oi >= 0) it[i] = lds_f32_unaligned(stage, r + oi);
        }
      }
    } else {
#pragma unroll
      for (int i = 0; i < IPT; ++i) {
        const uint32_t li = li0 + 32 * i;
        x[i] = y[i] = z[i] = it[i] = 0.f;
        if (li < n_here) {
          const uint8_t* r = base + (size_t)li * step;
          x[i] = ldg_f32_bytes(r + ox);
          y[i] = ldg_f32_bytes(r + oy);
          z[i] = ldg_f32_bytes(r + oz);
          if (oi >= 0) it[i] = ldg_f32_bytes(r + oi);
        }
      }
    }
  }
  K1_TRACE(0);
  if (OBOX) __syncthreads();

  float m[12];
#pragma unroll
  for (int k = 0; k < 12; ++k) m[k] = sg->m[k];
  const bool dense = sg->is_dense != 0;

  uint32_t keep_bits = 0;
  uint32_t ballots[IPT];
  uint32_t inv_run = 0;
  float mn0 = 3.402823466e+38f, mn1 = mn0, mn2 = mn0, mx0 = -mn0, mx1 = -mn0, mx2 = -mn0;
  const float lo0 = p.crop.lo[0], lo1 = p.crop.lo[1], lo2 = p.crop.lo[2], lo3 = p.crop.lo[3];
  const float hi0 = p.crop.hi[0], hi1 = p.crop.hi[1], hi2 = p.crop.hi[2], hi3 = p.crop.hi[3];
#pragma unroll
  for (int i = 0; i < IPT; ++i) {
    const bool in_range = full || (li0 + 32 * i < n_here);
    const float a = x[i], b = y[i], c = z[i];
    bool keep, fold;
    if (BOX) {
      x[i] = __fadd_rn(__fadd_rn(__fadd_rn(__fmul_rn(m[0], a), __fmul_rn(m[1], b)), __fmul_rn(m[2], c)), m[3]);
      y[i] = __fadd_rn(__fadd_rn(__fadd_rn(__fmul_rn(m[4], a), __fmul_rn(m[5], b)), __fmul_rn(m[6], c)), m[7]);
      z[i] = __fadd_rn(__fadd_rn(__fadd_rn(__fmul_rn(m[8], a), __fmul_rn(m[9], b)), __fmul_rn(m[10], c)), m[11]);
      keep = in_range & (x[i] >= lo0) & (x[i] <= hi0) & (y[i] >= lo1) & (y[i] <= hi1) & (z[i] >= lo2) & (z[i] <= hi2);
      if (BOX == 2) keep = keep & (it[i] >= lo3) & (it[i] <= hi3);
      if (OBOX && __any_sync(0xFFFFFFFFu, keep))
        for (uint32_t k = 0; k < n_obox; ++k) keep = keep & obox_keeps(sbox[k], x[i], y[i], z[i]);
      fold = keep;
    } else {
      const bool fin_in = finite_f32(a) && finite_f32(b) && finite_f32(c);
      if (dense || fin_in) {
        x[i] = __fadd_rn(__fadd_rn(__fadd_rn(__fmul_rn(m[0], a), __fmul_rn(m[1], b)), __fmul_rn(m[2], c)), m[3]);
        y[i] = __fadd_rn(__fadd_rn(__fadd_rn(__fmul_rn(m[4], a), __fmul_rn(m[5], b)), __fmul_rn(m[6], c)), m[7]);
        z[i] = __fadd_rn(__fadd_rn(__fadd_rn(__fmul_rn(m[8], a), __fmul_rn(m[9], b)), __fmul_rn(m[10], c)), m[11]);
      }
      const bool fin = finite_f32(x[i]) && finite_f32(y[i]) && finite_f32(z[i]);
      keep = in_range;
      const int n_pass = p.crop.n_pass;
      if (n_pass > 0) {
        keep = keep && fin;
        for (int k = 0; k < n_pass; ++k) keep = keep && pass_keeps(p.crop.pass[k], x[i], y[i], z[i], it[i]);
      }
      if (OBOX) {
        if (n_pass == 0 && !dense) keep = keep && fin;
        if (__any_sync(0xFFFFFFFFu, keep))
          for (uint32_t k = 0; k < n_obox; ++k) keep = keep & obox_keeps(sbox[k], x[i], y[i], z[i]);
      }
      fold = keep && fin;
      inv_run += __popc(__ballot_sync(0xFFFFFFFFu, keep && !fin));
    }
    minmax_if(fold, x[i], mn0, mx0);
    minmax_if(fold, y[i], mn1, mx1);
    minmax_if(fold, z[i], mn2, mx2);
    ballots[i] = __ballot_sync(0xFFFFFFFFu, keep);
    keep_bits |= (keep ? 1u : 0u) << i;
  }
  uint32_t warp_run = 0;
#pragma unroll
  for (int i = 0; i < IPT; ++i) warp_run += __popc(ballots[i]);

  const uint32_t e0 = __reduce_max_sync(0xFFFFFFFFu, ~f32_order_enc(__float_as_uint(mn0)));
  const uint32_t e1 = __reduce_max_sync(0xFFFFFFFFu, ~f32_order_enc(__float_as_uint(mn1)));
  const uint32_t e2 = __reduce_max_sync(0xFFFFFFFFu, ~f32_order_enc(__float_as_uint(mn2)));
  const uint32_t e3 = __reduce_max_sync(0xFFFFFFFFu, f32_order_enc(__float_as_uint(mx0)));
  const uint32_t e4 = __reduce_max_sync(0xFFFFFFFFu, f32_order_enc(__float_as_uint(mx1)));
  const uint32_t e5 = __reduce_max_sync(0xFFFFFFFFu, f32_order_enc(__float_as_uint(mx2)));
  if (lane == 0) {
    s_warp_tot[warp] = warp_run;
    s_warp_inv[warp] = inv_run;
    s_mm[warp][0] = e0; s_mm[warp][1] = e1; s_mm[warp][2] = e2;
    s_mm[warp][3] = e3; s_mm[warp][4] = e4; s_mm[warp][5] = e5;
  }
  K1_TRACE(1);
  __syncthreads();
  K1_TRACE(2);

  uint32_t tot, inv, pos;
  {
    const uint32_t c = lane < (uint32_t)WARPS ? s_warp_tot[lane] : 0u;
    const uint32_t incl = warp_incl_scan_u32(c);
    pos = __shfl_sync(0xFFFFFFFFu, incl - c, warp);
    tot = __shfl_sync(0xFFFFFFFFu, incl, 31);
    inv = 0;
    if (!BOX) inv = warp_sum_u32(lane < (uint32_t)WARPS ? s_warp_inv[lane] : 0u);
  }
  const uint32_t slot0 = sg->slot_base + pt0;
  if (warp == 0) {
    const uint32_t frame = sg->frame;
    if (lane == 0) {
      TileRec rec;
      rec.count = tot; rec.slot0 = slot0; rec.frame = frame; rec.dense0 = 0;
      *reinterpret_cast<uint4*>(p.tile_rec + tile) = *reinterpret_cast<const uint4*>(&rec);
      if (inv) {
        atomicAdd(&p.acc[frame].n_invalid, inv);
        atomicOr(&p.ctrl->has_invalid, 1u);
      }
    }
    if (tot > inv && lane < 6) {
      uint32_t e = s_mm[0][lane];
#pragma unroll
      for (int w = 1; w < WARPS; ++w) e = max(e, s_mm[w][lane]);
      FrameAcc* fa = p.acc + frame;
      atomicMax(lane < 3 ? &fa->nmin_enc[lane] : &fa->max_enc[lane - 3], e);
    }
  }
  K1_TRACE(3);

  pos += slot0;
  const uint32_t src0 = sg->src_base + pt0 + li0;
  const uint32_t lt = lanemask_lt();
  const bool want_src = p.surv_src != nullptr;
  const uint32_t fbits = KEYS ? (sg->frame << p.box.idx_bits) : 0u;
#pragma unroll
  for (int i = 0; i < IPT; ++i) {
    if (keep_bits & (1u << i)) {
      const uint32_t q = pos + __popc(ballots[i] & lt);
      p.surv_xyzi[q] = make_float4(x[i], y[i], z[i], it[i]);
      if (want_src) p.surv_src[q] = src0 + 32 * i;
      if (KEYS) {
        const uint32_t i0 = (uint32_t)(__float2int_rd(__fmul_rn(x[i], p.box.inv[0])) - p.box.min_b[0]);
        const uint32_t i1 = (uint32_t)(__float2int_rd(__fmul_rn(y[i], p.box.inv[1])) - p.box.min_b[1]);
        const uint32_t i2 = (uint32_t)(__float2int_rd(__fmul_rn(z[i], p.box.inv[2])) - p.box.min_b[2]);
        const uint32_t key = fbits | (i0 + i1 * p.box.mul1 + i2 * p.box.mul2);
        p.surv_key[q] = key;
        atomicAdd(&s_hist[key & (CM_RADIX - 1)], 1u);
      }
    }
    pos += __popc(ballots[i]);
  }
  if (KEYS) {
    __syncthreads();
    if (tid < CM_RADIX) {
      const uint32_t c = s_hist[tid];
      if (c) atomicAdd(p.hist + tid, c);
    }
  }
  K1_TRACE(5);
}

template <int THREADS, int IPT, bool OBOX>
cudaError_t launch_cfg(const K1Params& p, int mode, int box, uint32_t smem, cudaStream_t stream) {
  const bool keys = p.surv_key != nullptr && box != 0;
#define CM_K1_LAUNCH(MODE, BOX, KEYS) k_transform_crop<THREADS, IPT, MODE, BOX, KEYS, OBOX><<<p.n_tiles, THREADS, smem, stream>>>(p)
#define CM_K1_BOX(MODE) do { if (box == 1) { if (keys) CM_K1_LAUNCH(MODE, 1, true); else CM_K1_LAUNCH(MODE, 1, false); } \
                             else if (box == 2) { if (keys) CM_K1_LAUNCH(MODE, 2, true); else CM_K1_LAUNCH(MODE, 2, false); } \
                             else CM_K1_LAUNCH(MODE, 0, false); } while (0)
  if (mode == (int)SEG_PACKED16) CM_K1_BOX((int)SEG_PACKED16);
  else if (mode == (int)SEG_PCL32) CM_K1_BOX((int)SEG_PCL32);
  else CM_K1_BOX(MODE_GENERIC);
#undef CM_K1_BOX
#undef CM_K1_LAUNCH
  return cudaGetLastError();
}

}

uint32_t k1_tile_points(int64_t total_points) {
  static const int forced = getenv("CM_K1_TILE") ? atoi(getenv("CM_K1_TILE")) : 0;
  if (forced == 1024 || forced == 4096) return (uint32_t)forced;
  return total_points >= (int64_t)K1_BIG_BATCH_POINTS ? 4096u : 1024u;
}
uint32_t k1_min_tile_points() { return 1024u; }
uint32_t k1_staged_smem(uint32_t tile_points, uint32_t max_step) { return tile_points * max_step + 16u; }

cudaError_t configure_device_kernels() {
  const int big = 200 * 1024;
  const int small = (int)k1_staged_smem(1024u, CM_MAX_STAGED_STEP);
  cudaError_t e;
#define CM_K1_ATTR(T, I, B, K, BYTES)                                                                                            \
  e = cudaFuncSetAttribute(k_transform_crop<T, I, MODE_GENERIC, B, K, false>, cudaFuncAttributeMaxDynamicSharedMemorySize, BYTES); \
  if (e != cudaSuccess) return e;                                                                                                  \
  e = cudaFuncSetAttribute(k_transform_crop<T, I, MODE_GENERIC, B, K, true>, cudaFuncAttributeMaxDynamicSharedMemorySize, BYTES);  \
  if (e != cudaSuccess) return e;
  CM_K1_ATTR(512, 8, 0, false, big) CM_K1_ATTR(512, 8, 1, false, big) CM_K1_ATTR(512, 8, 2, false, big)
  CM_K1_ATTR(512, 8, 1, true, big) CM_K1_ATTR(512, 8, 2, true, big)
  CM_K1_ATTR(256, 4, 0, false, small) CM_K1_ATTR(256, 4, 1, false, small) CM_K1_ATTR(256, 4, 2, false, small)
  CM_K1_ATTR(256, 4, 1, true, small) CM_K1_ATTR(256, 4, 2, true, small)
#undef CM_K1_ATTR
  return cudaSuccess;
}

cudaError_t launch_transform_crop(const K1Params& p, uint32_t tile_points, int mode, uint32_t staged_smem_bytes,
                                  cudaStream_t stream) {
  if (p.n_tiles == 0) return cudaSuccess;
  const int box = p.crop.is_box ? (p.crop.use_i ? 2 : 1) : 0;
  if (p.n_obox) {
    if (tile_points == 4096u) return launch_cfg<512, 8, true>(p, mode, box, staged_smem_bytes, stream);
    return launch_cfg<256, 4, true>(p, mode, box, staged_smem_bytes, stream);
  }
  if (tile_points == 4096u) return launch_cfg<512, 8, false>(p, mode, box, staged_smem_bytes, stream);
  return launch_cfg<256, 4, false>(p, mode, box, staged_smem_bytes, stream);
}

}
```

### cloud_merger_b200/csrc/cm_voxel.cu

```cuda
#include "cm_kernels.h"

namespace cm {

namespace {

constexpr int VX_THREADS = 256;
constexpr int KH_IPT = 8;
constexpr int KH_TILE = VX_THREADS * KH_IPT;
constexpr int KH_DENSE_TILE = 4096;
constexpr int SCAN_THREADS = 1024;
#ifndef KH_UNROLL
#define KH_UNROLL 8
#endif
#ifndef CE_ASYNC_GATHER
#define CE_ASYNC_GATHER 1
#endif
#ifndef CE_MIN_CTAS
#define CE_MIN_CTAS (CE_ASYNC_GATHER ? 3 : 4)
#endif
#ifndef CE_PREFETCH
#define CE_PREFETCH 0
#endif
#ifndef CE_LB_POLL_ONE
#define CE_LB_POLL_ONE 0
// ... 33 lines not shown
}

}

__global__ void __launch_bounds__(VX_THREADS) k_minmax(const float4* __restrict__ pts, uint32_t n, Ctrl* ctrl,
                                                       FrameAcc* acc, uint32_t* frame_surv_start) {
  __shared__ float s_mm[VX_THREADS / 32][6];
  __shared__ uint32_t s_inv[VX_THREADS / 32];
  const uint32_t tid = threadIdx.x, lane = tid & 31u, warp = tid >> 5;
  float mn0 = 3.402823466e+38f, mn1 = mn0, mn2 = mn0, mx0 = -mn0, mx1 = -mn0, mx2 = -mn0;
  uint32_t inv = 0, fin_cnt = 0;
  for (size_t i = (size_t)blockIdx.x * VX_THREADS + tid; i < n; i += (size_t)gridDim.x * VX_THREADS) {
    const float4 v = ldg_stream_f4(pts + i);
    if (finite_f32(v.x) && finite_f32(v.y) && finite_f32(v.z)) {
      mn0 = fminf(mn0, v.x); mx0 = fmaxf(mx0, v.x);
      mn1 = fminf(mn1, v.y); mx1 = fmaxf(mx1, v.y);
      mn2 = fminf(mn2, v.z); mx2 = fmaxf(mx2, v.z);
      ++fin_cnt;
    } else {
      ++inv;
    }
  }
#pragma unroll
  for (int o = 16; o > 0; o >>= 1) {
    mn0 = fminf(mn0, __shfl_xor_sync(0xFFFFFFFFu, mn0, o)); mx0 = fmaxf(mx0, __shfl_xor_sync(0xFFFFFFFFu, mx0, o));
    mn1 = fminf(mn1, __shfl_xor_sync(0xFFFFFFFFu, mn1, o)); mx1 = fmaxf(mx1, __shfl_xor_sync(0xFFFFFFFFu, mx1, o));
    mn2 = fminf(mn2, __shfl_xor_sync(0xFFFFFFFFu, mn2, o)); mx2 = fmaxf(mx2, __shfl_xor_sync(0xFFFFFFFFu, mx2, o));
  }
  inv = warp_sum_u32(inv);
  fin_cnt = warp_sum_u32(fin_cnt);
  if (lane == 0) {
    s_mm[warp][0] = mn0; s_mm[warp][1] = mn1; s_mm[warp][2] = mn2;
    s_mm[warp][3] = mx0; s_mm[warp][4] = mx1; s_mm[warp][5] = mx2;
    s_inv[warp] = inv;
    if (fin_cnt == 0) s_mm[warp][0] = 3.402823466e+38f;
  }
  __syncthreads();
  if (tid == 0) {
    float a0 = s_mm[0][0], a1 = s_mm[0][1], a2 = s_mm[0][2], b0 = s_mm[0][3], b1 = s_mm[0][4], b2 = s_mm[0][5];
    uint32_t ti = s_inv[0];
    for (int w = 1; w < VX_THREADS / 32; ++w) {
      a0 = fminf(a0, s_mm[w][0]); a1 = fminf(a1, s_mm[w][1]); a2 = fminf(a2, s_mm[w][2]);
      b0 = fmaxf(b0, s_mm[w][3]); b1 = fmaxf(b1, s_mm[w][4]); b2 = fmaxf(b2, s_mm[w][5]);
      ti += s_inv[w];
    }
    if (b0 >= a0) {
      atomicMax(&acc->nmin_enc[0], ~f32_order_enc(__float_as_uint(a0)));
      atomicMax(&acc->nmin_enc[1], ~f32_order_enc(__float_as_uint(a1)));
      atomicMax(&acc->nmin_enc[2], ~f32_order_enc(__float_as_uint(a2)));
      atomicMax(&acc->max_enc[0], f32_order_enc(__float_as_uint(b0)));
      atomicMax(&acc->max_enc[1], f32_order_enc(__float_as_uint(b1)));
      atomicMax(&acc->max_enc[2], f32_order_enc(__float_as_uint(b2)));
    }
    if (ti) {
      atomicAdd(&acc->n_invalid, ti);
      atomicOr(&ctrl->has_invalid, 1u);
    }
    if (blockIdx.x == 0) {
      frame_surv_start[0] = 0;
      frame_surv_start[1] = n;
    }
  }
}

__device__ __forceinline__ void tile_scan_body(TileRec* __restrict__ rec, uint32_t n_tiles, const SegDev* __restrict__ segs,
                                               uint32_t n_seg, uint32_t n_frames, uint32_t* frame_surv_start,
                                               uint32_t* seg_surv_start, uint32_t* s_scr ) {
  const uint32_t tid = threadIdx.x;
  const uint32_t chunk = (n_tiles + SCAN_THREADS - 1) / SCAN_THREADS;
  const uint32_t b = min(n_tiles, tid * chunk), e = min(n_tiles, b + chunk);
  constexpr int W = 8;
  uint32_t c[W];
  uint32_t sum = 0;
  for (uint32_t i0 = b; i0 < e; i0 += W) {
#pragma unroll
    for (int k = 0; k < W; ++k) c[k] = (i0 + k < e) ? rec[i0 + k].count : 0u;
#pragma unroll
    for (int k = 0; k < W; ++k) sum += c[k];
  }
  uint32_t total;
  uint32_t run = block_excl_scan_1024(sum, s_scr, &total);
  if (chunk <= (uint32_t)W) {
#pragma unroll
    for (int k = 0; k < W; ++k) {
      if (b + k < e) rec[b + k].dense0 = run;
      run += c[k];
    }
  } else {
    for (uint32_t i = b; i < e; ++i) {
      const uint32_t cc = rec[i].count;
      rec[i].dense0 = run;
      run += cc;
    }
  }
  __syncthreads();
  for (uint32_t s = tid; s < n_seg; s += SCAN_THREADS) {
    const uint32_t d0 = rec[segs[s].tile_begin].dense0;
    seg_surv_start[s] = d0;
    if (segs[s].first_of_frame) frame_surv_start[segs[s].frame] = d0;
  }
  if (tid == 0) frame_surv_start[n_frames] = total;
}

__global__ void __launch_bounds__(SCAN_THREADS) k_tile_scan(TileRec* __restrict__ rec, uint32_t n_tiles,
                                                           const SegDev* __restrict__ segs, uint32_t n_seg,
                                                           uint32_t n_frames, uint32_t* frame_surv_start,
                                                           uint32_t* seg_surv_start) {
  __shared__ uint32_t s_scr[33];
  tile_scan_body(rec, n_tiles, segs, n_seg, n_frames, frame_surv_start, seg_surv_start, s_scr);
}

__global__ void __launch_bounds__(VX_THREADS) k_compact_survivors(const TileRec* __restrict__ rec, uint32_t n_tiles,
                                                                 const float4* __restrict__ slot_xyzi,
                                                                 const uint32_t* __restrict__ slot_src,
                                                                 float4* __restrict__ dense_xyzi,
                                                                 uint32_t* __restrict__ dense_src,
                                                                 uint32_t* __restrict__ dense_slot) {
  for (uint32_t t = blockIdx.x; t < n_tiles; t += gridDim.x) {
    const TileRec r = rec[t];
    for (uint32_t j = threadIdx.x; j < r.count; j += VX_THREADS) {
      dense_xyzi[r.dense0 + j] = slot_xyzi[r.slot0 + j];
      if (dense_src) dense_src[r.dense0 + j] = slot_src[r.slot0 + j];
      if (dense_slot) dense_slot[r.dense0 + j] = r.slot0 + j;
    }
  }
}

__global__ void k_seed_bounds(FrameAcc* acc, float mn0, float mn1, float mn2, float mx0, float mx1, float mx2) {
  if (threadIdx.x == 0 && blockIdx.x == 0) {
    atomicMax(&acc->nmin_enc[0], ~f32_order_enc(__float_as_uint(mn0)));
    atomicMax(&acc->nmin_enc[1], ~f32_order_enc(__float_as_uint(mn1)));
    atomicMax(&acc->nmin_enc[2], ~f32_order_enc(__float_as_uint(mn2)));
    atomicMax(&acc->max_enc[0], f32_order_enc(__float_as_uint(mx0)));
    atomicMax(&acc->max_enc[1], f32_order_enc(__float_as_uint(mx1)));
    atomicMax(&acc->max_enc[2], f32_order_enc(__float_as_uint(mx2)));
  }
}

struct TileScanArgs {
  TileRec* rec;
  uint32_t n_tiles;
  const SegDev* segs;
  uint32_t n_seg;
  uint32_t* seg_surv_start;
};
__global__ void __launch_bounds__(SCAN_THREADS) k_grid_setup(const VoxelParams p, const TileScanArgs ts) {
  __shared__ uint32_t s_maxbits;
  __shared__ uint32_t s_scr[33];
  const uint32_t tid = threadIdx.x;
  if (tid == 0) s_maxbits = 0;
  if (ts.rec) tile_scan_body(ts.rec, ts.n_tiles, ts.segs, ts.n_seg, p.n_frames, const_cast<uint32_t*>(p.frame_surv_start),
                             ts.seg_surv_start, s_scr);
  __syncthreads();
  if (ts.rec && p.fused_keys) {
    const unsigned long long T = p.sort_tile;
    for (uint32_t i = tid; i < ts.n_tiles; i += SCAN_THREADS) {
      const uint32_t c = ts.rec[i].count;
      if (!c) continue;
      const unsigned long long d0 = ts.rec[i].dense0;
      const unsigned long long t = (d0 + T - 1ull) / T;
      if (t * T < d0 + c) p.first_k1[t] = i;
    }
  }
  for (uint32_t f = tid; f < p.n_frames; f += SCAN_THREADS) {
    const FrameAcc a = p.acc[f];
    GridDev g;
    g.pcl_overflow = 0;
    g.bits = 0;
    g.mul1 = 0;
    g.mul2 = 0;
    g.zero_keys = 0;
    g.empty = (a.max_enc[0] == 0u && a.nmin_enc[0] == 0u) ? 1u : 0u;
    if (g.empty) {
      for (int k = 0; k < 3; ++k) { g.min_b[k] = 0; g.max_b[k] = 0; g.div_b[k] = 0; }
    } else {
      long long d[3];
      unsigned long long div[3];
      bool range_err = false;
      for (int k = 0; k < 3; ++k) {
        const float mn = __uint_as_float(f32_order_dec(~a.nmin_enc[k]));
        const float mx = __uint_as_float(f32_order_dec(a.max_enc[k]));
        const float inv = p.inv_leaf[k];
        d[k] = __float2ll_rz(__fmul_rn(__fsub_rn(mx, mn), inv)) + 1ll;
        const float fmn = floorf(__fmul_rn(mn, inv)), fmx = floorf(__fmul_rn(mx, inv));
        if (!(fabsf(fmn) < 1073741824.f) || !(fabsf(fmx) < 1073741824.f)) range_err = true;
        g.min_b[k] = (int)fmn;
        g.max_b[k] = (int)fmx;
        const long long dv = (long long)g.max_b[k] - (long long)g.min_b[k] + 1ll;
        g.div_b[k] = (int)dv;
        div[k] = (unsigned long long)dv;
        if (dv > (1ll << 21)) range_err = true;
      }
      const long long imax = 2147483647ll;
      bool ovf = d[0] > imax || d[1] > imax || d[2] > imax || d[0] < 0 || d[1] < 0 || d[2] < 0;
      if (!ovf) {
        const long long p01 = d[0] * d[1];
        ovf = p01 > imax || p01 * d[2] > imax;
      }
      g.pcl_overflow = ovf ? 1 : 0;
      if (range_err) {
        if (!(p.pcl_refuses && ovf)) atomicExch(&p.ctrl->error, (uint32_t)CM_DEV_E_KEY_RANGE);
        div[0] = div[1] = div[2] = 1;
        g.zero_keys = 1;
      }
      g.mul1 = div[0];
      g.mul2 = div[0] * div[1];
      const unsigned long long cells = div[0] * div[1] * div[2];
      g.bits = cells <= 1ull ? 0u : (uint32_t)(64 - __clzll((long long)(cells - 1ull)));
      atomicMax(&s_maxbits, g.bits);
    }
    p.grid[f] = g;
  }
  __syncthreads();
  {
    const uint32_t e = *p.epoch_dev;
    const bool wrap = e + 64u >= (1u << 30);
    if (wrap) {
      for (uint32_t i = tid; i < p.lb_sort_words; i += SCAN_THREADS) p.lb_sort[i] = 0ull;
      for (uint32_t i = tid; i < p.cent_status_words; i += SCAN_THREADS) p.cent_status[i] = 0ull;
    }
    __syncthreads();
    if (tid == 0) *p.epoch_dev = wrap ? 16u : e + 16u;
  }
  __shared__ SortInfo s_si;
  if (tid == 0) {
    const bool has_invalid = p.ctrl->has_invalid != 0u;
    const uint32_t key_frames = p.n_frames + (has_invalid ? 1u : 0u);
    uint32_t frame_bits = key_frames <= 1u ? 0u : (uint32_t)(32 - __clz((int)(key_frames - 1u)));
    uint32_t idx_bits = s_maxbits;
    if (p.fused_keys) idx_bits = p.box.idx_bits;
    bool seg = p.segmented == 2u;
    if (p.segmented == 1u) seg = !has_invalid && idx_bits <= 32u;
    if (seg) frame_bits = 0u;
    uint32_t width = p.key_bytes;
    if (p.dual_width) width = p.segmented == 1u ? (seg ? 4u : 8u) : (frame_bits + idx_bits <= 32u ? 4u : 8u);
    uint32_t total = frame_bits + idx_bits;
    if (total > width * 8u) {
      atomicExch(&p.ctrl->error, (uint32_t)CM_DEV_E_KEY_RANGE);
      total = width * 8u;
      idx_bits = total - frame_bits;
    }
    uint32_t passes = (total + CM_RADIX_BITS - 1) / CM_RADIX_BITS;
    if (passes == 0) passes = 1;
    if (passes > p.max_passes) {
      atomicExch(&p.ctrl->error, (uint32_t)CM_DEV_E_KEY_RANGE);
      passes = p.max_passes;
    }
    SortInfo si;
    si.num_passes = passes;
    si.total_bits = total;
    si.idx_bits = idx_bits;
    si.n_keys = p.frame_surv_start[p.n_frames];
    si.key_frames = key_frames;
    si.width = width;
    si.segmented = seg ? 1u : 0u;
    si.n_seg_tiles = 0;
    s_si = si;
  }
  __syncthreads();
  if (s_si.segmented) {
    const uint32_t T = p.sort_tile, F = p.n_frames;
    uint32_t carry = 0;
    for (uint32_t f0 = 0; f0 < F; f0 += SCAN_THREADS) {
      const uint32_t f = f0 + tid;
      const uint32_t nf = f < F ? p.frame_surv_start[f + 1] - p.frame_surv_start[f] : 0u;
      uint32_t tot;
      const uint32_t ex = block_excl_scan_1024((nf + T - 1u) / T, s_scr, &tot);
      if (f < F) p.seg_frame_tile0[f] = carry + ex;
      carry += tot;
    }
    if (tid == 0) { p.seg_frame_tile0[F] = carry; s_si.n_seg_tiles = carry; }
    __syncthreads();
    const uint32_t warp = tid >> 5, lane = tid & 31u;
    for (uint32_t f = warp; f < F; f += SCAN_THREADS / 32) {
      const uint32_t b = p.frame_surv_start[f], e = p.frame_surv_start[f + 1];
      const uint32_t t0 = p.seg_frame_tile0[f], nt = p.seg_frame_tile0[f + 1] - t0;
      for (uint32_t t = lane; t < nt; t += 32u) {
        SegTile st;
        st.base = b + t * T;
        st.n = min(T, e - st.base);
        st.frame = f | (t == 0u ? CM_SEG_FIRST : 0u);
        st.pad = 0u;
        p.seg_tile[t0 + t] = st;
      }
    }
    const uint32_t M = s_si.n_keys;
    auto frame_from = [&](uint32_t i, uint32_t lo) {
      uint32_t hi = F - 1u;
      while (lo < hi) {
        const uint32_t mid = (lo + hi + 1u) >> 1;
        if (p.frame_surv_start[mid] <= i) lo = mid; else hi = mid - 1u;
      }
      return lo;
    };
    for (uint32_t t = tid; (unsigned long long)t * CE_TILE < M; t += SCAN_THREADS) {
      const uint32_t b = t * CE_TILE, e = min(b + (uint32_t)CE_TILE, M);
      const uint32_t lo = frame_from(b, 0u);
      p.seg_cent_range[t] = make_uint2(lo, frame_from(e - 1u, lo));
    }
    __syncthreads();
  }
  if (tid == 0) *p.info = s_si;
}

template <typename KeyT, bool CHECK, bool SEG = false>
__device__ __forceinline__ void key_hist_tiles(const VoxelParams& p, uint32_t (*s_hist)[CM_RADIX], const SortInfo& si,
                                               uint32_t M) {
  const uint32_t tid = threadIdx.x;
  const uint32_t F = p.n_frames;
  const uint32_t n_pass = si.num_passes, idx_bits = si.idx_bits;
  const bool dense = p.tile_rec == nullptr;
  uint32_t n_tiles = p.n_k1_tiles;
  if (dense) {
    n_tiles = 0;
    for (uint32_t f = 0; f < F; ++f)
      n_tiles += (p.frame_surv_start[f + 1] - p.frame_surv_start[f] + KH_DENSE_TILE - 1) / KH_DENSE_TILE;
  }
  KeyT* __restrict__ keys = reinterpret_cast<KeyT*>(p.keys_a);
  uint32_t* __restrict__ vals = p.vals_a;
  uint2* __restrict__ recs = reinterpret_cast<uint2*>(p.keys_a);
  const unsigned long long sentinel = (unsigned long long)F << idx_bits;
  const float inv0 = p.inv_leaf[0], inv1 = p.inv_leaf[1], inv2 = p.inv_leaf[2];

  uint32_t hist_frame = 0xFFFFFFFFu;
  auto flush_frame = [&]() {
    __syncthreads();
    if (hist_frame != 0xFFFFFFFFu) {
      uint32_t* dst = p.seg_hist + (size_t)hist_frame * (CM_SEG_PASSES * CM_RADIX);
      for (uint32_t i = tid; i < n_pass * CM_RADIX; i += VX_THREADS) {
        const uint32_t c = (&s_hist[0][0])[i];
        if (c) { atomicAdd(dst + i, c); (&s_hist[0][0])[i] = 0u; }
      }
    }
    __syncthreads();
  };
  for (uint32_t tile = blockIdx.x; tile < n_tiles; tile += gridDim.x) {
    TileRec r;
    if (dense) {
      uint32_t t = tile, f = 0, f_begin = 0, f_end = 0;
      for (; f < F; ++f) {
        f_begin = p.frame_surv_start[f]; f_end = p.frame_surv_start[f + 1];
        const uint32_t tf = (f_end - f_begin + KH_DENSE_TILE - 1) / KH_DENSE_TILE;
        if (t < tf) break;
        t -= tf;
      }
      r.frame = f; r.slot0 = f_begin + t * KH_DENSE_TILE; r.dense0 = r.slot0;
      r.count = min((uint32_t)KH_DENSE_TILE, f_end - r.slot0);
    } else {
      const uint4 q = __ldg(reinterpret_cast<const uint4*>(p.tile_rec + tile));
      r.count = q.x; r.slot0 = q.y; r.frame = q.z; r.dense0 = q.w;
    }
    if (r.count == 0) continue;
    if (SEG && r.frame != hist_frame) {
      flush_frame();
      hist_frame = r.frame;
    }
    const GridDev* __restrict__ g = p.grid + r.frame;
    const KeyT fbits = SEG ? (KeyT)0 : (KeyT)((unsigned long long)r.frame << idx_bits);
    const KeyT mul1 = (KeyT)g->mul1, mul2 = (KeyT)g->mul2;
    const KeyT idx_keep = g->zero_keys ? (KeyT)0 : ~(KeyT)0;
    const int mb0 = g->min_b[0], mb1 = g->min_b[1], mb2 = g->min_b[2];
    const float4* __restrict__ src = p.pts + r.slot0;
    constexpr int U = KH_UNROLL;
    for (uint32_t j0 = 0; j0 < r.count; j0 += U * VX_THREADS) {
      const bool whole = j0 + U * VX_THREADS <= r.count;
      float4 pv[U];
      if (whole) {
#pragma unroll
        for (int u = 0; u < U; ++u) pv[u] = ldg_stream_f4(src + j0 + u * VX_THREADS + tid);
      } else {
#pragma unroll
        for (int u = 0; u < U; ++u) {
          const uint32_t j = j0 + u * VX_THREADS + tid;
          pv[u] = (j < r.count) ? ldg_stream_f4(src + j) : make_float4(0.f, 0.f, 0.f, 0.f);
        }
      }
#pragma unroll
      for (int u = 0; u < U; ++u) {
        const uint32_t j = j0 + u * VX_THREADS + tid;
        if (!whole && j >= r.count) continue;
        const float4 v = pv[u];
        const KeyT i0 = (KeyT)(__float2int_rd(__fmul_rn(v.x, inv0)) - mb0);
        const KeyT i1 = (KeyT)(__float2int_rd(__fmul_rn(v.y, inv1)) - mb1);
        const KeyT i2 = (KeyT)(__float2int_rd(__fmul_rn(v.z, inv2)) - mb2);
        KeyT key = fbits | ((KeyT)(i0 + i1 * mul1 + i2 * mul2) & idx_keep);
        if (CHECK && !(finite_f32(v.x) && finite_f32(v.y) && finite_f32(v.z))) key = (KeyT)sentinel;
        if (sizeof(KeyT) == 4) {
          recs[r.dense0 + j] = make_uint2((uint32_t)key, r.slot0 + j);
        } else {
          keys[r.dense0 + j] = key;
          vals[r.dense0 + j] = r.slot0 + j;
        }
        if (sizeof(KeyT) == 4) {
#pragma unroll
          for (uint32_t ps = 0; ps < 4; ++ps)
            if (ps < n_pass) atomicAdd(&s_hist[ps][((uint32_t)key >> (ps * CM_RADIX_BITS)) & (CM_RADIX - 1)], 1u);
        } else {
#pragma unroll
          for (uint32_t ps = 0; ps < CM_MAX_SORT_PASSES; ++ps)
            if (ps < n_pass)
              atomicAdd(&s_hist[ps][(uint32_t)((unsigned long long)key >> (ps * CM_RADIX_BITS)) & (CM_RADIX - 1)], 1u);
        }
      }
    }
  }
  if (SEG) flush_frame();
}

template <typename KeyT>
__global__ void __launch_bounds__(VX_THREADS) k_voxel_key_hist(const VoxelParams p) {
  __shared__ uint32_t s_hist[CM_MAX_SORT_PASSES][CM_RADIX];
  const uint32_t tid = threadIdx.x;
  const SortInfo si = *p.info;
  if (p.dual_width && ((si.width == 4u) != (sizeof(KeyT) == 4))) return;
  for (uint32_t i = tid; i < CM_MAX_SORT_PASSES * CM_RADIX; i += VX_THREADS) (&s_hist[0][0])[i] = 0;
  __syncthreads();
  const uint32_t M = p.frame_surv_start[p.n_frames];
  if (sizeof(KeyT) == 4 && si.segmented) {
    key_hist_tiles<uint32_t, false, true>(p, s_hist, si, M);
    return;
  }
  if (si.key_frames > p.n_frames) key_hist_tiles<KeyT, true>(p, s_hist, si, M);
  else key_hist_tiles<KeyT, false>(p, s_hist, si, M);
  __syncthreads();
  for (uint32_t i = tid; i < si.num_passes * CM_RADIX; i += VX_THREADS) {
    const uint32_t c = (&s_hist[0][0])[i];
    if (c) atomicAdd(p.hist + i, c);
  }
}

__global__ void __launch_bounds__(CM_RADIX) k_seg_base(const VoxelParams p) {
  __shared__ uint32_t s_scan[12];
  const SortInfo si = *p.info;
  if (!si.segmented || blockIdx.y >= si.num_passes) return;
  const uint32_t f = blockIdx.x, tid = threadIdx.x;
  uint32_t* h = p.seg_hist + ((size_t)f * CM_SEG_PASSES + blockIdx.y) * CM_RADIX;
  uint32_t tot;
  const uint32_t ex = block_excl_scan_256(h[tid], s_scan, &tot);
  h[tid] = p.frame_surv_start[f] + ex;
}

__global__ void __launch_bounds__(VX_THREADS) k_seg_keys64(const uint2* __restrict__ rec, unsigned long long* __restrict__ keys,
                                                          uint32_t* __restrict__ vals, const VoxelParams p) {
  const uint32_t F = p.n_frames, idx_bits = p.info->idx_bits;
  const uint32_t* __restrict__ fss = p.frame_surv_start;
  const uint32_t n = fss[F];
  for (uint32_t i = blockIdx.x * VX_THREADS + threadIdx.x; i < n; i += gridDim.x * VX_THREADS) {
    uint32_t lo = 0, hi = F - 1u;
    while (lo < hi) {
      const uint32_t mid = (lo + hi + 1u) >> 1;
      if (fss[mid] <= i) lo = mid; else hi = mid - 1u;
    }
    const uint2 r = rec[i];
    keys[i] = ((unsigned long long)lo << idx_bits) | (unsigned long long)r.x;
    vals[i] = r.y;
  }
}

constexpr uint32_t CE_TAIL_INLINE = 24;
constexpr int CE_TAIL_U = 4;
constexpr int CE_TAIL_ITEMS = CE_TAIL_U * VX_THREADS;
struct TailRun {
  float sx, sy, sz, sw;
  unsigned long long key;
  uint32_t n, dst, g;
  uint32_t count_frame;
};
template <typename KeyT, bool SEG>
__device__ __noinline__ void finish_tail_run(const VoxelParams* pp, const TailRun* tr_s, float4* s_pts, uint32_t* s_lead) {
  constexpr bool REC = SEG || sizeof(KeyT) == 4;
  const VoxelParams& p = *pp;
  const TailRun tr = *tr_s;
  const uint32_t tid = threadIdx.x, lane = tid & 31u;
  const SortInfo si = *p.info;
  const uint32_t F = p.n_frames, idx_bits = si.idx_bits;
  const bool odd = (si.num_passes & 1u) != 0u;
  const void* __restrict__ sorted = odd ? p.keys_b : p.keys_a;
  const uint32_t* __restrict__ vals = odd ? p.vals_b : p.vals_a;
  uint32_t limit = p.frame_surv_start[F];
  unsigned long long want = tr.key;
  if (SEG) {
    limit = p.frame_surv_start[(tr.key >> idx_bits) + 1ull];
    want = tr.key & ((1ull << idx_bits) - 1ull);
  }
  float sx = tr.sx, sy = tr.sy, sz = tr.sz, sw = tr.sw;
  uint32_t n = tr.n, g = tr.g;
  while (true) {
#pragma unroll 1
    for (int u = 0; u < CE_TAIL_U; ++u) {
      const uint32_t i = g + (uint32_t)u * VX_THREADS + tid;
      bool m = i < limit && i >= g;
      uint32_t slot = 0;
      if (m) {
        if (REC) {
          const uint2 r = reinterpret_cast<const uint2*>(sorted)[i];
          m = (unsigned long long)r.x == want;
          slot = r.y;
        } else {
          m = (unsigned long long)reinterpret_cast<const KeyT*>(sorted)[i] == want;
          slot = vals[i];
        }
      }
      const uint32_t bal = __ballot_sync(0xFFFFFFFFu, m);
      if (lane == 0) s_lead[u * (VX_THREADS / 32) + (tid >> 5)] = bal == 0xFFFFFFFFu ? 32u : (uint32_t)__ffs(~bal) - 1u;
      if (m) s_pts[u * VX_THREADS + tid] = __ldg(p.pts + slot);
    }
    __syncthreads();
    uint32_t matched = 0;
    bool open = true;
#pragma unroll 1
    for (int w = 0; w < CE_TAIL_U * (VX_THREADS / 32); ++w) {
      const uint32_t l = s_lead[w];
      matched += open ? l : 0u;
      open = open && l == 32u;
    }
    if (tid == 0) {
      for (uint32_t q = 0; q < matched; ++q) {
        const float4 pt = s_pts[q];
        sx = __fadd_rn(sx, pt.x); sy = __fadd_rn(sy, pt.y); sz = __fadd_rn(sz, pt.z); sw = __fadd_rn(sw, pt.w);
      }
    }
    n += matched;
    g += matched;
    __syncthreads();
    if (matched < (uint32_t)CE_TAIL_ITEMS) break;
  }
  if (tid == 0) {
    const float nf = (float)n;
    const float4 c = make_float4(__fdiv_rn(sx, nf), __fdiv_rn(sy, nf), __fdiv_rn(sz, nf), p.downsample_all ? __fdiv_rn(sw, nf) : 0.f);
    if (p.out_step == 32) {
      float4* o = reinterpret_cast<float4*>(reinterpret_cast<uint8_t*>(p.out_xyzi) + (size_t)tr.dst * 32);
      o[0] = make_float4(c.x, c.y, c.z, 1.0f);
      o[1] = make_float4(c.w, 0.f, 0.f, 0.f);
    } else {
      reinterpret_cast<float4*>(p.out_xyzi)[tr.dst] = c;
    }
    p.out_count[tr.dst] = n;
    const unsigned long long f = idx_bits >= 64 ? 0ull : tr.key >> idx_bits;
    unsigned long long vidx = idx_bits >= 64 ? tr.key : tr.key & ((1ull << idx_bits) - 1ull);
    if (p.fused_keys) {
      const uint32_t b = (uint32_t)vidx;
      const uint32_t k2 = b / p.box.mul2, r2 = b - k2 * p.box.mul2;
      const uint32_t k1 = r2 / p.box.mul1, k0 = r2 - k1 * p.box.mul1;
      const GridDev* __restrict__ gd = p.grid + (f < F ? f : 0ull);
      const long long c0 = (long long)k0 + p.box.min_b[0] - gd->min_b[0];
      const long long c1 = (long long)k1 + p.box.min_b[1] - gd->min_b[1];
      const long long c2 = (long long)k2 + p.box.min_b[2] - gd->min_b[2];
      vidx = (unsigned long long)(c0 + c1 * (long long)gd->mul1 + c2 * (long long)gd->mul2);
    }
    p.out_idx[tr.dst] = vidx;
    if (tr.count_frame && f < F) atomicAdd(&p.acc[f].voxel_count, 1u);
  }
}

constexpr uint32_t CE_SEG_SMEM_FRAMES = 256;
template <typename KeyT, bool SEG = false>
__global__ void __launch_bounds__(VX_THREADS, CE_MIN_CTAS) k_voxel_centroid(const VoxelParams p) {
  static_assert(!SEG || sizeof(KeyT) == 8, "the logical key of a segmented run is 64 bits wide");
  constexpr bool REC = SEG || sizeof(KeyT) == 4;
  __shared__ uint32_t s_fss[SEG ? CE_SEG_SMEM_FRAMES + 1 : 1];
  __shared__ uint32_t s_scan[9];
  extern __shared__ __align__(16) float4 s_pts_buf[];
  __shared__ uint32_t s_headw[CE_TILE / 32 + 1];
  __shared__ unsigned short s_start[CE_TILE];
  __shared__ uint32_t s_tile, s_base;
  __shared__ uint32_t s_cnt8[VX_THREADS / 32];
  __shared__ VoxelParams s_params;
  __shared__ TailRun s_tail;
  __shared__ uint32_t s_tail_r;
  __shared__ uint32_t s_tail_lead[CE_TAIL_U * (VX_THREADS / 32)];
  const uint32_t tid = threadIdx.x, lane = tid & 31u;
  const uint32_t F = p.n_frames;
  const uint32_t M = p.frame_surv_start[F];
  const uint32_t n_tiles = (M + CE_TILE - 1) / CE_TILE;
  if (p.dual_width && ((p.info->width == 4u) != REC)) return;
  if (SEG != (p.info->segmented != 0u)) return;
  if (tid == 0) s_tile = atomicAdd(&p.ctrl->cent_ticket, 1u);
  __syncthreads();
  uint32_t tile = s_tile;
  if (tile >= n_tiles) return;
  for (uint32_t i = tid; i < sizeof(VoxelParams) / 4; i += VX_THREADS)
    reinterpret_cast<uint32_t*>(&s_params)[i] = reinterpret_cast<const uint32_t*>(&p)[i];

  const SortInfo si = *p.info;
  const uint32_t idx_bits = si.idx_bits;
  const bool odd = (si.num_passes & 1u) != 0u;
  const uint32_t epoch = *p.epoch_dev + 9u;
  const void* __restrict__ sorted = odd ? p.keys_b : p.keys_a;
  const uint32_t* __restrict__ vals = odd ? p.vals_b : p.vals_a;
  const bool fss_staged = SEG && F <= CE_SEG_SMEM_FRAMES;
  if (fss_staged) {
    for (uint32_t i = tid; i <= F; i += VX_THREADS) s_fss[i] = p.frame_surv_start[i];
// ... 279 lines not shown
    for (q = s0; q < end; ++q) {
      const float4 pt = s_pts[q];
      sx = __fadd_rn(sx, pt.x); sy = __fadd_rn(sy, pt.y); sz = __fadd_rn(sz, pt.z); sw = __fadd_rn(sw, pt.w);
    }
    uint32_t n = end - s0;
    if (end == tile_n) {
      uint32_t g = tile_base + tile_n;
      while (g < M && key_at(g) == key) {
        if (g - (tile_base + tile_n) == CE_TAIL_INLINE) {
          s_tail.sx = sx; s_tail.sy = sy; s_tail.sz = sz; s_tail.sw = sw;
          s_tail.key = (unsigned long long)key; s_tail.n = n; s_tail.g = g;
          s_tail_r = r;
          return false;
        }
        const float4 pt = __ldg(p.pts + val_at(g));
        sx = __fadd_rn(sx, pt.x); sy = __fadd_rn(sy, pt.y); sz = __fadd_rn(sz, pt.z); sw = __fadd_rn(sw, pt.w);
        ++n; ++g;
      }
    }
    if (n == 1u) {
      cen = make_float4(sx, sy, sz, p.downsample_all ? sw : 0.f);
    } else {
      const float nf = (float)n;
      cen = make_float4(__fdiv_rn(sx, nf), __fdiv_rn(sy, nf), __fdiv_rn(sz, nf), p.downsample_all ? __fdiv_rn(sw, nf) : 0.f);
    }
    n_out = n;
    key_out = key;
    return true;
  };
  auto emit = [&](uint32_t dst, const float4& c, uint32_t n, KeyT key) {
    if (p.out_step == 32) {
      float4* o = reinterpret_cast<float4*>(reinterpret_cast<uint8_t*>(p.out_xyzi) + (size_t)dst * 32);
      o[0] = make_float4(c.x, c.y, c.z, 1.0f);
      o[1] = make_float4(c.w, 0.f, 0.f, 0.f);
    } else {
      reinterpret_cast<float4*>(p.out_xyzi)[dst] = c;
    }
    p.out_count[dst] = n;
    unsigned long long vidx = (unsigned long long)key & idx_mask;
    if (p.fused_keys) {
      const uint32_t b = (uint32_t)vidx;
      const uint32_t k2 = b / p.box.mul2, r2 = b - k2 * p.box.mul2;
      const uint32_t k1 = r2 / p.box.mul1, k0 = r2 - k1 * p.box.mul1;
      const unsigned long long f = (unsigned long long)key >> idx_bits;
      const GridDev* __restrict__ g = p.grid + (f < F ? f : 0ull);
      const long long c0 = (long long)k0 + p.box.min_b[0] - g->min_b[0];
      const long long c1 = (long long)k1 + p.box.min_b[1] - g->min_b[1];
      const long long c2 = (long long)k2 + p.box.min_b[2] - g->min_b[2];
      vidx = (unsigned long long)(c0 + c1 * (long long)g->mul1 + c2 * (long long)g->mul2);
    }
    p.out_idx[dst] = vidx;
    if (per_voxel_count) {
      const unsigned long long f = (unsigned long long)key >> idx_bits;
      if (f < F) atomicAdd(&p.acc[f].voxel_count, 1u);
    }
  };
  float4 c0 = make_float4(0.f, 0.f, 0.f, 0.f);
  uint32_t n0 = 0;
  KeyT k0 = (KeyT)0;
  bool whole0 = false;
  if (tid < total) whole0 = voxel(tid, c0, n0, k0);
  __syncthreads();
  const uint32_t out0 = s_base;
  if (whole0) emit(out0 + tid, c0, n0, k0);
  for (uint32_t r = tid + VX_THREADS; r < total; r += VX_THREADS)
    if (voxel(r, c0, n0, k0)) emit(out0 + r, c0, n0, k0);
  __syncthreads();
  if (s_tail_r != 0xFFFFFFFFu) {
    if (tid == 0) {
      s_tail.dst = out0 + s_tail_r;
      s_tail.count_frame = per_voxel_count ? 1u : 0u;
    }
    __syncthreads();
    finish_tail_run<KeyT, SEG>(&s_params, &s_tail, s_pts, s_tail_lead);
    __syncthreads();
  }
  tile = next_tile;
  head = next_head;
  pass = next_pass;
  buf = next_buf;
  if (tile >= n_tiles) break;
  }
}

__global__ void __launch_bounds__(VX_THREADS) k_export_voxels(const VoxelParams p, uint4* __restrict__ host_xyzi,
                                                             uint32_t* __restrict__ host_count,
                                                             unsigned long long* __restrict__ host_idx, uint32_t cap) {
  const uint32_t V = min(p.ctrl->total_voxels, cap);
  const uint32_t stride = gridDim.x * VX_THREADS, t0 = blockIdx.x * VX_THREADS + threadIdx.x;
  const uint32_t n16 = V * (p.out_step / 16u);
  const uint4* __restrict__ sx = reinterpret_cast<const uint4*>(p.out_xyzi);
  for (uint32_t i = t0; i < n16; i += stride) host_xyzi[i] = sx[i];
  const uint4* __restrict__ sc = reinterpret_cast<const uint4*>(p.out_count);
  for (uint32_t i = t0; i < V / 4u; i += stride) reinterpret_cast<uint4*>(host_count)[i] = sc[i];
  const uint4* __restrict__ si = reinterpret_cast<const uint4*>(p.out_idx);
  for (uint32_t i = t0; i < V / 2u; i += stride) reinterpret_cast<uint4*>(host_idx)[i] = si[i];
  if (blockIdx.x == 0) {
    for (uint32_t i = (V & ~3u) + threadIdx.x; i < V; i += VX_THREADS) host_count[i] = p.out_count[i];
    for (uint32_t i = (V & ~1u) + threadIdx.x; i < V; i += VX_THREADS) host_idx[i] = p.out_idx[i];
  }
}

static inline uint32_t persistent_grid(uint32_t n_tiles) {
  const uint32_t cap = 148u * 8u;
  return n_tiles < 1u ? 1u : (n_tiles < cap ? n_tiles : cap);
}

cudaError_t launch_minmax(const float4* pts, uint32_t n, Ctrl* ctrl, FrameAcc* acc, uint32_t* frame_surv_start,
                          cudaStream_t stream) {
  const uint32_t tiles = (n + KH_TILE - 1) / KH_TILE;
  k_minmax<<<persistent_grid(tiles), VX_THREADS, 0, stream>>>(pts, n, ctrl, acc, frame_surv_start);
  return cudaGetLastError();
}

cudaError_t launch_seed_bounds(FrameAcc* acc, const float* mn, const float* mx, cudaStream_t stream) {
  k_seed_bounds<<<1, 32, 0, stream>>>(acc, mn[0], mn[1], mn[2], mx[0], mx[1], mx[2]);
  return cudaGetLastError();
}

cudaError_t launch_tile_scan(TileRec* tile_rec, uint32_t n_tiles, const SegDev* segs, uint32_t n_seg, uint32_t n_frames,
                             uint32_t* frame_surv_start, uint32_t* seg_surv_start, cudaStream_t stream) {
  k_tile_scan<<<1, SCAN_THREADS, 0, stream>>>(tile_rec, n_tiles, segs, n_seg, n_frames, frame_surv_start, seg_surv_start);
  return cudaGetLastError();
}

cudaError_t launch_compact_survivors(const TileRec* tile_rec, uint32_t n_tiles, const float4* slot_xyzi,
                                     const uint32_t* slot_src, float4* dense_xyzi, uint32_t* dense_src,
                                     uint32_t* dense_slot, cudaStream_t stream) {
  if (n_tiles == 0) return cudaSuccess;
  k_compact_survivors<<<persistent_grid(n_tiles), VX_THREADS, 0, stream>>>(tile_rec, n_tiles, slot_xyzi, slot_src,
                                                                            dense_xyzi, dense_src, dense_slot);
  return cudaGetLastError();
}

cudaError_t launch_grid_setup(const VoxelParams& p, cudaStream_t stream, TileRec* scan_rec, uint32_t scan_tiles,
                              const SegDev* segs, uint32_t n_seg, uint32_t* seg_surv_start) {
  TileScanArgs ts;
  ts.rec = scan_rec; ts.n_tiles = scan_tiles; ts.segs = segs; ts.n_seg = n_seg; ts.seg_surv_start = seg_surv_start;
  k_grid_setup<<<1, SCAN_THREADS, 0, stream>>>(p, ts);
  return cudaGetLastError();
}

cudaError_t launch_key_hist(const VoxelParams& p, cudaStream_t stream) {
  const uint32_t tiles = p.tile_rec ? p.n_k1_tiles : (p.max_points + KH_DENSE_TILE - 1) / KH_DENSE_TILE + p.n_frames;
  if (p.key_bytes == 4)
    k_voxel_key_hist<uint32_t><<<persistent_grid(tiles), VX_THREADS, 0, stream>>>(p);
  else
    k_voxel_key_hist<unsigned long long><<<persistent_grid(tiles), VX_THREADS, 0, stream>>>(p);
  return cudaGetLastError();
}

cudaError_t launch_seg_base(const VoxelParams& p, cudaStream_t stream) {
  if (p.n_frames == 0) return cudaSuccess;
  k_seg_base<<<dim3(p.n_frames, CM_SEG_PASSES), CM_RADIX, 0, stream>>>(p);
  return cudaGetLastError();
}

cudaError_t launch_seg_keys64(const void* records, unsigned long long* keys, uint32_t* vals, const VoxelParams& p,
                              cudaStream_t stream) {
  if (p.max_points == 0) return cudaSuccess;
  const uint32_t blocks = std::min<uint32_t>((p.max_points + VX_THREADS - 1u) / VX_THREADS, 148u * 8u);
  k_seg_keys64<<<blocks, VX_THREADS, 0, stream>>>(reinterpret_cast<const uint2*>(records), keys, vals, p);
  return cudaGetLastError();
}

cudaError_t launch_centroid(const VoxelParams& p, cudaStream_t stream) {
  const uint32_t tiles = (p.max_points + CE_TILE - 1) / CE_TILE;
  if (tiles == 0) return cudaSuccess;
  const uint32_t grid = std::min<uint32_t>(tiles, 148u * (uint32_t)CE_MIN_CTAS);
  if (p.key_bytes == 4 && p.segmented)
    k_voxel_centroid<unsigned long long, true><<<grid, VX_THREADS, CE_DYN_SMEM, stream>>>(p);
  else if (p.key_bytes == 4)
    k_voxel_centroid<uint32_t><<<grid, VX_THREADS, CE_DYN_SMEM, stream>>>(p);
  else
    k_voxel_centroid<unsigned long long><<<grid, VX_THREADS, CE_DYN_SMEM, stream>>>(p);
  return cudaGetLastError();
}

cudaError_t configure_centroid_kernels() {
  cudaError_t e = cudaFuncSetAttribute(k_voxel_centroid<unsigned long long, true>, cudaFuncAttributeMaxDynamicSharedMemorySize,
                                       (int)CE_DYN_SMEM);
  if (e == cudaSuccess)
    e = cudaFuncSetAttribute(k_voxel_centroid<uint32_t>, cudaFuncAttributeMaxDynamicSharedMemorySize, (int)CE_DYN_SMEM);
  if (e == cudaSuccess)
    e = cudaFuncSetAttribute(k_voxel_centroid<unsigned long long>, cudaFuncAttributeMaxDynamicSharedMemorySize, (int)CE_DYN_SMEM);
  return e;
}

cudaError_t launch_export_voxels(const VoxelParams& p, void* host_xyzi, uint32_t* host_count, unsigned long long* host_idx,
                                 uint32_t cap, cudaStream_t stream) {
  const uint32_t blocks = std::max(1u, std::min<uint32_t>(148u, (cap + 4u * VX_THREADS - 1u) / (4u * VX_THREADS)));
  k_export_voxels<<<blocks, VX_THREADS, 0, stream>>>(p, static_cast<uint4*>(host_xyzi), host_count, host_idx, cap);
  return cudaGetLastError();
}

uint32_t centroid_tile_items() { return CE_TILE; }

}
```

Baseline: 49770.

## Sort fused box keys per frame with a wide top digit to drop a radix pass

When crop-box keys are fused, the keys are now sorted segment by segment per frame rather than with frame bits prepended. The top digit may use up to 384 bins so that one fewer 8-bit onesweep pass is needed. Per-frame histograms are collected in the crop kernel, the fused first pass counts later digits per frame, and a segment-base scan runs after pass 0. This adds per-frame histogram flushes, wider shared-memory scans and more scanner CTAs, and it is easy to get subtly wrong.

Measured after the change: 51850, median of 6. 4.2% higher.

```diff
diff --git a/cloud_merger_b200/csrc/cm_api.cu b/cloud_merger_b200/csrc/cm_api.cu
--- a/cloud_merger_b200/csrc/cm_api.cu
+++ b/cloud_merger_b200/csrc/cm_api.cu
@@ -333,15 +333,15 @@
   CM_CUDA(h, dev_alloc(w.surv_xyzi, np));
   CM_CUDA(h, dev_alloc(w.surv_src, np));
   CM_CUDA(h, dev_alloc(w.surv_key, np));
-  CM_CUDA(h, dev_alloc(w.first_k1, sort_lookback_rows((uint32_t)np)));
+  CM_CUDA(h, dev_alloc(w.first_k1, sort_lookback_rows((uint32_t)np) + frames));
   CM_CUDA(h, dev_alloc(w.keys_a, np, 0));
   CM_CUDA(h, dev_alloc(w.keys_b, np, 0));
   CM_CUDA(h, dev_alloc(w.vals_a, np));
   CM_CUDA(h, dev_alloc(w.vals_b, np));
   w.lb_k1_n = np / k1_min_tile_points() + segs + 2;
   CM_CUDA(h, dev_alloc(w.tile_seg, w.lb_k1_n));
-  w.lb_sort_n = (sort_lookback_rows((uint32_t)np) + (frames > 1 ? frames : 0u)) * CM_RADIX;
-  if (frames > 1) {
+  w.lb_sort_n = (sort_lookback_rows((uint32_t)np) + frames) * CM_WIDE_BINS;
+  {
     CM_CUDA(h, dev_alloc(w.seg_tile, sort_lookback_rows((uint32_t)np) + frames));
     CM_CUDA(h, dev_alloc(w.seg_hist, (size_t)frames * CM_SEG_PASSES * CM_RADIX));
     CM_CUDA(h, dev_alloc(w.seg_frame_tile0, (size_t)frames + 1));
@@ -442,6 +442,19 @@
   g->mul2 = (uint32_t)(div[0] * div[1]);
   g->idx_bits = idx_bits;
   g->n_pass = std::max<uint32_t>(1u, (bits + CM_RADIX_BITS - 1) / CM_RADIX_BITS);
+  static const bool no_wide = getenv("CM_NO_WIDE_TOP") != nullptr;
+  g->seg_sort = 0;
+  g->top_bins = CM_RADIX;
+  if (!no_wide && cells > CM_WIDE_BINS) {
+    uint32_t p = 2;
+    unsigned long long span = CM_RADIX;
+    while ((cells + span - 1) / span > CM_WIDE_BINS) { ++p; span *= CM_RADIX; }
+    if (p < g->n_pass) {
+      g->n_pass = p;
+      g->seg_sort = 1;
+      g->top_bins = (cells + span - 1) / span > CM_RADIX ? CM_WIDE_BINS : CM_RADIX;
+    }
+  }
   return true;
 }
 
@@ -579,6 +592,10 @@
       CM_CUDA(h, cudaEventRecord(w.ev[EV_SORT0].get(), st));
       w.timed_pass0 = true;
     }
+    if (ps == 0 && vp.fused_keys && vp.box.seg_sort && vp.max_passes > 1) {
+      CM_CUDA(h, launch_seg_base(vp, st));
+      ++w.launches;
+    }
   }
   if (h->profiling) CM_CUDA(h, cudaEventRecord(w.ev[EV_SORT].get(), st));
   if (!with_centroid) {
@@ -726,6 +743,12 @@
   w.fused_keys = fused; w.box = box;
   kp.surv_key = fused ? w.surv_key.get() : nullptr;
   kp.hist = reinterpret_cast<uint32_t*>(w.meta.get() + w.ml.off_hist);
+  kp.hist_frame_stride = 0;
+  if (fused && box.seg_sort) {
+    CM_CUDA(h, cudaMemsetAsync(w.seg_hist.get(), 0, (size_t)n_frames * CM_SEG_PASSES * CM_RADIX * sizeof(uint32_t), st));
+    kp.hist = w.seg_hist.get();
+    kp.hist_frame_stride = CM_SEG_PASSES * CM_RADIX;
+  }
   kp.box = box;
   kp.obox = nullptr; kp.n_obox = 0;
   if (h->n_obox > 0) {
diff --git a/cloud_merger_b200/csrc/cm_common.cuh b/cloud_merger_b200/csrc/cm_common.cuh
--- a/cloud_merger_b200/csrc/cm_common.cuh
+++ b/cloud_merger_b200/csrc/cm_common.cuh
@@ -130,6 +130,7 @@
   uint32_t width;
   uint32_t segmented;
   uint32_t n_seg_tiles;
+  uint32_t seg_sort;
 };
 
 struct SegTile {
@@ -140,6 +141,7 @@
 };
 constexpr uint32_t CM_SEG_FIRST = 0x80000000u;
 constexpr uint32_t CM_SEG_PASSES = 4;
+constexpr uint32_t CM_WIDE_BINS = 384;
 
 __host__ __device__ __forceinline__ uint32_t f32_order_enc(uint32_t bits) {
   return bits ^ ((bits >> 31) ? 0xFFFFFFFFu : 0x80000000u);
@@ -249,28 +251,33 @@
   }
 }
 
-__device__ __forceinline__ uint32_t block_excl_scan_256(uint32_t v, uint32_t* scratch, uint32_t* total) {
+template <int N>
+__device__ __forceinline__ uint32_t block_excl_scan(uint32_t v, uint32_t* scratch, uint32_t* total) {
+  constexpr int W = N / 32;
   const uint32_t tid = threadIdx.x, lane = tid & 31u, w = tid >> 5;
-  if (tid >= 256) v = 0;
+  if (tid >= (uint32_t)N) v = 0;
   const uint32_t incl = warp_incl_scan_u32(v);
-  if (lane == 31 && w < 8) scratch[w] = incl;
+  if (lane == 31 && w < W) scratch[w] = incl;
   __syncthreads();
   if (tid == 0) {
     uint32_t run = 0;
 #pragma unroll
-    for (int i = 0; i < 8; ++i) {
+    for (int i = 0; i < W; ++i) {
       uint32_t t = scratch[i];
       scratch[i] = run;
       run += t;
     }
-    scratch[8] = run;
+    scratch[W] = run;
   }
   __syncthreads();
-  const uint32_t res = incl - v + (w < 8 ? scratch[w] : 0u);
-  *total = scratch[8];
+  const uint32_t res = incl - v + (w < W ? scratch[w] : 0u);
+  *total = scratch[W];
   __syncthreads();
   return res;
 }
+__device__ __forceinline__ uint32_t block_excl_scan_256(uint32_t v, uint32_t* scratch, uint32_t* total) {
+  return block_excl_scan<256>(v, scratch, total);
+}
 
 #endif
 
diff --git a/cloud_merger_b200/csrc/cm_kernels.h b/cloud_merger_b200/csrc/cm_kernels.h
--- a/cloud_merger_b200/csrc/cm_kernels.h
+++ b/cloud_merger_b200/csrc/cm_kernels.h
@@ -13,6 +13,8 @@
   uint32_t mul1, mul2;
   uint32_t idx_bits;
   uint32_t n_pass;
+  uint32_t seg_sort;
+  uint32_t top_bins;
 };
 struct K1Params {
   const SegDev* segs;
@@ -28,6 +30,7 @@
   FrameAcc* acc;
   uint32_t* surv_key;
   uint32_t* hist;
+  uint32_t hist_frame_stride;
   BoxGrid box;
   TileRec* tile_rec;
   unsigned long long* trace;
diff --git a/cloud_merger_b200/csrc/cm_radix_sort.cu b/cloud_merger_b200/csrc/cm_radix_sort.cu
--- a/cloud_merger_b200/csrc/cm_radix_sort.cu
+++ b/cloud_merger_b200/csrc/cm_radix_sort.cu
@@ -37,19 +37,20 @@
   static constexpr int IPT = RS_IPT64;
 };
 
-constexpr int RS_SCANNERS = 8;
-constexpr int RS_SCAN_DIGITS = CM_RADIX / RS_SCANNERS;
+constexpr int RS_SCAN_DIGITS = 32;
+constexpr int RS_SCANNERS = CM_RADIX / RS_SCAN_DIGITS;
 constexpr int RS_SCAN_ROWS = 32;
 constexpr int RS_SCAN_GROUP = RS_THREADS >= 512 ? 8 : 16;
-static_assert(RS_SCAN_DIGITS == 32, "one digit per lane");
-
-template <bool SEG>
+static_assert(RS_THREADS >= (int)CM_WIDE_BINS, "one thread per digit of a wide pass is needed");
+
+template <bool SEG, int NB = CM_RADIX>
 __device__ __forceinline__ void scanner_cta(uint32_t scanner , unsigned long long* rows ,
                                             uint32_t n_tiles, uint32_t epoch, const uint32_t* hist ,
                                             uint32_t* err, uint32_t* s_scan, uint32_t* s_tmp ,
                                             unsigned long long* s_chain , const SegTile* __restrict__ seg_tile,
                                             const uint32_t* __restrict__ seg_base ) {
   const uint32_t tid = threadIdx.x, lane = tid & 31u, q = tid >> 5;
+  static_assert(SEG || NB == CM_RADIX, "a wide top digit is only ranked frame by frame");
   const uint32_t d = scanner * RS_SCAN_DIGITS + lane;
   if (SEG) {
     if (q == 0) s_chain[lane] = 0ull;
@@ -69,7 +70,7 @@
   volatile unsigned long long* chain = s_chain + lane;
   for (uint32_t b = q; b < n_batches; b += RS_WARPS) {
     const uint32_t r0 = b * RS_SCAN_ROWS;
-    unsigned long long* const base = rows + (size_t)r0 * CM_RADIX + d;
+    unsigned long long* const base = rows + (size_t)r0 * NB + d;
     uint32_t c[RS_SCAN_ROWS];
 #pragma unroll
     for (int g0 = 0; g0 < RS_SCAN_ROWS; g0 += RS_SCAN_GROUP) {
@@ -79,7 +80,7 @@
         unsigned long long w[RS_SCAN_GROUP];
 #pragma unroll
         for (int k = 0; k < RS_SCAN_GROUP; ++k)
-          w[k] = (r0 + g0 + k < n_tiles) ? ld_cg_u64(base + (size_t)(g0 + k) * CM_RADIX) : lb_pack(epoch, CM_LB_AGG, 0u);
+          w[k] = (r0 + g0 + k < n_tiles) ? ld_cg_u64(base + (size_t)(g0 + k) * NB) : lb_pack(epoch, CM_LB_AGG, 0u);
         bool all = true;
 #pragma unroll
         for (int k = 0; k < RS_SCAN_GROUP; ++k) {
@@ -132,12 +133,12 @@
 #pragma unroll
       for (int k = 0; k < RS_SCAN_ROWS; ++k)
         if (r0 + k < n_tiles)
-          st_cg_u64(base + (size_t)k * CM_RADIX, lb_pack(epoch, CM_LB_INCL, (uint32_t)k >= abs_from ? c[k] : run + c[k]));
+          st_cg_u64(base + (size_t)k * NB, lb_pack(epoch, CM_LB_INCL, (uint32_t)k >= abs_from ? c[k] : run + c[k]));
     } else {
       *chain = ((unsigned long long)(b + 1u) << 32) | (unsigned long long)(run + sum);
 #pragma unroll
       for (int k = 0; k < RS_SCAN_ROWS; ++k)
-        if (r0 + k < n_tiles) st_cg_u64(base + (size_t)k * CM_RADIX, lb_pack(epoch, CM_LB_INCL, run + c[k]));
+        if (r0 + k < n_tiles) st_cg_u64(base + (size_t)k * NB, lb_pack(epoch, CM_LB_INCL, run + c[k]));
     }
   }
 }
@@ -159,40 +160,67 @@
   return a | c;
 }
 
+template <int BITS>
+__device__ __forceinline__ uint32_t warp_diff(uint32_t x) {
+  if constexpr (BITS == 8) {
+    return warp_diff8(x);
+  } else {
+    static_assert(BITS == 9, "8 or 9 digit bits");
+    const uint32_t t8 = warp_diff8(x);
+    uint32_t t;
+    asm volatile(
+        "{\n .reg .pred p;\n .reg .b32 y;\n and.b32 y, %1, %2;\n setp.ne.u32 p, y, 0;\n"
+        " vote.sync.ballot.b32 %0, p, 0xffffffff;\n @p not.b32 %0, %0;\n}"
+        : "=r"(t)
+        : "r"(x), "r"(1u << 8));
+    return t8 | t;
+  }
+}
+
+template <int NB, typename KeyT>
+__device__ __forceinline__ uint32_t sort_digit(KeyT k, uint32_t shift, uint32_t idx_mask) {
+  if constexpr (NB == CM_RADIX) return (uint32_t)(k >> shift) & (CM_RADIX - 1);
+  else return min(((uint32_t)k & idx_mask) >> shift, (uint32_t)NB - 1u);
+}
+
 __device__ __forceinline__ uint32_t lanemask_gt() {
   uint32_t m;
   asm("mov.u32 %0, %%lanemask_gt;" : "=r"(m));
   return m;
 }
 
-template <typename KeyT, int IPT>
+template <typename KeyT, int IPT, int NB = CM_RADIX, bool WIDE_LATER = false>
 struct SortSmem {
   static constexpr int TILE = RS_THREADS * IPT;
   static constexpr bool AOS = sizeof(KeyT) == 4;
+  static constexpr int LATER = 3 * CM_RADIX + (WIDE_LATER ? (int)CM_WIDE_BINS - CM_RADIX : 0);
   unsigned long long k[2][TILE];
   uint32_t v[2][AOS ? 1 : TILE];
-  uint32_t hist[RS_WARPS * CM_RADIX];
-  uint32_t scatter[2][CM_RADIX];
-  uint32_t scan[12];
-  uint32_t cnt[CM_RADIX];
-  uint32_t later[3][CM_RADIX];
+  uint32_t hist[RS_WARPS * NB];
+  uint32_t scatter[2][NB];
+  uint32_t scan[NB / 32 + 4];
+  uint32_t cnt[NB];
+  uint32_t later[LATER];
   uint32_t next_tile[2];
 };
 
-template <typename KeyT, int IPT, bool FUSED0 = false, bool SEG = false>
+template <typename KeyT, int IPT, bool FUSED0 = false, bool SEG = false, int NB = CM_RADIX>
 __global__ void __launch_bounds__(RS_THREADS, RS_MIN_CTAS) k_onesweep_pass(const VoxelParams p, const int pass) {
-  static_assert(!SEG || (sizeof(KeyT) == 4 && !FUSED0), "segmented keys are 32-bit records written by k_voxel_key_hist");
+  static_assert(!SEG || sizeof(KeyT) == 4, "segmented keys are 32-bit records");
+  static_assert(NB == CM_RADIX || (SEG && !FUSED0 && NB == (int)CM_WIDE_BINS), "a wide digit is the top digit of a SEG run");
   constexpr int TILE = RS_THREADS * IPT;
   constexpr int WARP_ITEMS = 32 * IPT;
   constexpr bool AOS = sizeof(KeyT) == 4;
+  constexpr int SCANNERS = NB / RS_SCAN_DIGITS;
+  using Smem = SortSmem<KeyT, IPT, NB, FUSED0 && SEG>;
   extern __shared__ __align__(16) unsigned char s_raw[];
-  SortSmem<KeyT, IPT>& sm = *reinterpret_cast<SortSmem<KeyT, IPT>*>(s_raw);
+  Smem& sm = *reinterpret_cast<Smem*>(s_raw);
 
   const long long tr0 = clock64();
   const SortInfo si = *p.info;
   if ((uint32_t)pass >= si.num_passes) return;
   if (p.dual_width && ((si.width == 4u) != (sizeof(KeyT) == 4))) return;
-  if (SEG != (si.segmented != 0u)) return;
+  if (SEG != (si.seg_sort != 0u)) return;
   const uint32_t M = si.n_keys;
   const uint32_t n_tiles = SEG ? si.n_seg_tiles : (M + TILE - 1) / TILE;
   const uint32_t* const seg_base = SEG ? p.seg_hist + (size_t)pass * CM_RADIX : nullptr;
@@ -200,19 +228,19 @@
   const uint32_t tid = threadIdx.x, lane = tid & 31u;
   const uint32_t warp = __shfl_sync(0xFFFFFFFFu, tid >> 5, 0);
   const uint32_t epoch = *p.epoch_dev + 1u + (uint32_t)pass;
-  unsigned long long* const rows = p.lb_sort + CM_RADIX;
+  unsigned long long* const rows = p.lb_sort + NB;
   uint32_t* const err = &p.ctrl->error;
   uint32_t* const counter = &p.ctrl->tile_counter[1 + pass];
   if (tid == 0) {
     const uint32_t role = atomicAdd(&p.ctrl->role_counter[pass], 1u);
     sm.next_tile[1] = role;
-    if (role >= (uint32_t)RS_SCANNERS) sm.next_tile[0] = atomicAdd(counter, 1u);
+    if (role >= (uint32_t)SCANNERS) sm.next_tile[0] = atomicAdd(counter, 1u);
   }
   __syncthreads();
   const uint32_t role = sm.next_tile[1];
-  if (role < (uint32_t)RS_SCANNERS) {
+  if (role < (uint32_t)SCANNERS) {
     __syncthreads();
-    scanner_cta<SEG>(role, rows, n_tiles, epoch, p.hist + pass * CM_RADIX, err, sm.scan, sm.hist, &sm.k[0][0], p.seg_tile, seg_base);
+    scanner_cta<SEG, NB>(role, rows, n_tiles, epoch, p.hist + pass * CM_RADIX, err, sm.scan, sm.hist, &sm.k[0][0], p.seg_tile, seg_base);
     return;
   }
 
@@ -220,11 +248,21 @@
   const bool odd = (pass & 1) != 0;
   const uint32_t shift = (uint32_t)pass * CM_RADIX_BITS;
   const uint32_t lt = lanemask_lt(), gt = lanemask_gt();
-  uint32_t* const wh = sm.hist + warp * CM_RADIX;
-
-  if (RS_EARLY_COUNT && tid < CM_RADIX) sm.cnt[tid] = 0;
+  uint32_t* const wh = sm.hist + warp * NB;
+  const uint32_t idx_mask = (NB > CM_RADIX || (FUSED0 && SEG)) ? (si.idx_bits >= 32u ? 0xFFFFFFFFu : (1u << si.idx_bits) - 1u) : 0u;
+  uint32_t hist_frame = 0xFFFFFFFFu;
+  auto flush_later = [&]() {
+    if (hist_frame == 0xFFFFFFFFu) return;
+    uint32_t* dst = p.seg_hist + (size_t)hist_frame * (CM_SEG_PASSES * CM_RADIX) + CM_RADIX;
+    for (uint32_t i = tid; i < (uint32_t)Smem::LATER; i += RS_THREADS) {
+      const uint32_t c = sm.later[i];
+      if (c) { atomicAdd(dst + i, c); sm.later[i] = 0u; }
+    }
+  };
+
+  if (RS_EARLY_COUNT && tid < NB) sm.cnt[tid] = 0;
   if (FUSED0)
-    for (uint32_t i = tid; i < 3u * CM_RADIX; i += RS_THREADS) (&sm.later[0][0])[i] = 0u;
+    for (uint32_t i = tid; i < (uint32_t)Smem::LATER; i += RS_THREADS) sm.later[i] = 0u;
   uint32_t cur = sm.next_tile[0];
   __syncthreads();
   uint32_t prev = 0xFFFFFFFFu, prev_n = 0;
@@ -251,6 +289,11 @@
       KeyT key[IPT];
       uint32_t val[IPT];
       if (FUSED0) {
+        if (SEG && (cur_seg & ~CM_SEG_FIRST) != hist_frame) {
+          flush_later();
+          hist_frame = cur_seg & ~CM_SEG_FIRST;
+          __syncthreads();
+        }
         const uint32_t k1_first = p.first_k1[cur];
         const uint32_t e = k1_first + lane;
         uint32_t e_dense = 0xFFFFFFFFu, e_slot = 0u, e_end = 0xFFFFFFFFu;
@@ -284,16 +327,32 @@
             }
             slot = tdense[lo * 4u + 1u] + (d - tdense[lo * 4u + 3u]);
           }
-          const bool in = d < M;
+          const bool in = SEG ? item0 + 32 * i < n_here : d < M;
           key[i] = in ? (KeyT)p.surv_key[slot] : ~(KeyT)0;
           val[i] = in ? slot : 0u;
         }
-#pragma unroll
-        for (int i = 0; i < IPT; ++i) {
-          if (tile_base + item0 + 32 * i < M) {
-#pragma unroll
-            for (uint32_t ps = 1; ps < 4; ++ps)
-              if (ps < si.num_passes) atomicAdd(&sm.later[ps - 1][((uint32_t)key[i] >> (ps * CM_RADIX_BITS)) & (CM_RADIX - 1)], 1u);
+        if (SEG) {
+          const uint32_t wide_pass = p.box.top_bins > CM_RADIX ? si.num_passes - 1u : 0u;
+#pragma unroll
+          for (int i = 0; i < IPT; ++i) {
+            if (item0 + 32 * i < n_here) {
+#pragma unroll
+              for (uint32_t ps = 1; ps < 3; ++ps)
+                if (ps < si.num_passes) {
+                  const uint32_t dg = ps == wide_pass ? sort_digit<(int)CM_WIDE_BINS>((uint32_t)key[i], ps * CM_RADIX_BITS, idx_mask)
+                                                      : sort_digit<CM_RADIX>((uint32_t)key[i], ps * CM_RADIX_BITS, 0u);
+                  atomicAdd(&sm.later[(ps - 1) * CM_RADIX + dg], 1u);
+                }
+            }
+          }
+        } else {
+#pragma unroll
+          for (int i = 0; i < IPT; ++i) {
+            if (tile_base + item0 + 32 * i < M) {
+#pragma unroll
+              for (uint32_t ps = 1; ps < 4; ++ps)
+                if (ps < si.num_passes) atomicAdd(&sm.later[(ps - 1) * CM_RADIX + (((uint32_t)key[i] >> (ps * CM_RADIX_BITS)) & (CM_RADIX - 1))], 1u);
+            }
           }
         }
       } else if (AOS) {
@@ -330,28 +389,35 @@
         }
       }
 #pragma unroll
-      for (int k = 0; k < CM_RADIX / 32; ++k) wh[lane + 32 * k] = 0;
+      for (int k = 0; k < NB / 32; ++k) wh[lane + 32 * k] = 0;
       __syncwarp();
       RS_TRACE(cur, 0, tr_cur);
       if (RS_EARLY_COUNT) {
 #pragma unroll
-        for (int i = 0; i < IPT; ++i) atomicAdd(&sm.cnt[(uint32_t)(key[i] >> shift) & (CM_RADIX - 1)], 1u);
+        for (int i = 0; i < IPT; ++i) atomicAdd(&sm.cnt[sort_digit<NB>(key[i], shift, idx_mask)], 1u);
         __syncthreads();
-        if (RS_THREADS == CM_RADIX || tid < CM_RADIX) {
+        if (RS_THREADS == NB || tid < NB) {
           const uint32_t c = sm.cnt[tid];
           sm.cnt[tid] = 0;
-          const uint32_t real = (tid == CM_RADIX - 1) ? c - ((uint32_t)TILE - n_here) : c;
-          st_relaxed_u64(rows + (size_t)cur * CM_RADIX + tid, lb_pack(epoch, CM_LB_AGG, real));
+          const uint32_t real = (tid == NB - 1) ? c - ((uint32_t)TILE - n_here) : c;
+          st_relaxed_u64(rows + (size_t)cur * NB + tid, lb_pack(epoch, CM_LB_AGG, real));
         }
       }
 
       uint32_t rank[IPT];
 #pragma unroll
       for (int i = 0; i < IPT; ++i) {
-        const uint32_t ks = (uint32_t)(key[i] >> shift);
-        const uint32_t diff = warp_diff8(ks);
+        uint32_t ks, diff;
+        if constexpr (NB == CM_RADIX) {
+          ks = (uint32_t)(key[i] >> shift);
+          diff = warp_diff<8>(ks);
+          ks &= CM_RADIX - 1;
+        } else {
+          ks = sort_digit<NB>(key[i], shift, idx_mask);
+          diff = warp_diff<9>(ks);
+        }
         const uint32_t below = (uint32_t)__popc(~diff & lt);
-        volatile uint32_t* c = wh + (ks & (CM_RADIX - 1));
+        volatile uint32_t* c = wh + ks;
         const uint32_t r = *c + below;
         rank[i] = r;
         if ((~diff & gt) == 0u) *c = r + 1u;
@@ -361,28 +427,28 @@
       RS_TRACE(cur, 1, tr_cur);
 
       {
-        const bool dt = RS_THREADS == CM_RADIX || tid < CM_RADIX;
+        const bool dt = RS_THREADS == NB || tid < NB;
         uint32_t wc[RS_WARPS];
         uint32_t cnt = 0;
         if (dt) {
 #pragma unroll
           for (int w = 0; w < RS_WARPS; ++w) {
-            wc[w] = sm.hist[w * CM_RADIX + tid];
+            wc[w] = sm.hist[w * NB + tid];
             cnt += wc[w];
           }
           if (!RS_EARLY_COUNT) {
-            const uint32_t real = (tid == CM_RADIX - 1) ? cnt - ((uint32_t)TILE - n_here) : cnt;
-            st_relaxed_u64(rows + (size_t)cur * CM_RADIX + tid, lb_pack(epoch, CM_LB_AGG, real));
+            const uint32_t real = (tid == NB - 1) ? cnt - ((uint32_t)TILE - n_here) : cnt;
+            st_relaxed_u64(rows + (size_t)cur * NB + tid, lb_pack(epoch, CM_LB_AGG, real));
           }
         }
         RS_TRACE(cur, 2, tr_cur);
         uint32_t tot;
-        const uint32_t bin_start = block_excl_scan_256(cnt, sm.scan, &tot);
+        const uint32_t bin_start = block_excl_scan<NB>(cnt, sm.scan, &tot);
         if (dt) {
           uint32_t run = bin_start;
 #pragma unroll
           for (int w = 0; w < RS_WARPS; ++w) {
-            sm.hist[w * CM_RADIX + tid] = run;
+            sm.hist[w * NB + tid] = run;
             run += wc[w];
           }
           sm.scatter[buf][tid] = 0u - bin_start;
@@ -393,8 +459,7 @@
 
 #pragma unroll
       for (int i = 0; i < IPT; ++i) {
-        const uint32_t ks = (uint32_t)(key[i] >> shift);
-        const uint32_t pos = wh[ks & (CM_RADIX - 1)] + rank[i];
+        const uint32_t pos = wh[sort_digit<NB>(key[i], shift, idx_mask)] + rank[i];
         if (AOS) {
           sm.k[buf][pos] = ((unsigned long long)val[i] << 32) | (unsigned long long)key[i];
         } else {
@@ -407,12 +472,12 @@
     if (prev != 0xFFFFFFFFu) {
       const uint32_t pb = buf ^ 1u;
       RS_TRACE(prev, 7, tr_prev);
-      if (RS_THREADS == CM_RADIX || tid < CM_RADIX) {
+      if (RS_THREADS == NB || tid < NB) {
         uint32_t first;
         if (SEG && (prev_seg & CM_SEG_FIRST))
           first = __ldg(seg_base + (size_t)(prev_seg & ~CM_SEG_FIRST) * (CM_SEG_PASSES * CM_RADIX) + tid);
         else
-          first = lb_wait_inclusive(rows + ((long long)prev - 1) * CM_RADIX + tid, epoch, err);
+          first = lb_wait_inclusive(rows + ((long long)prev - 1) * NB + tid, epoch, err);
         sm.scatter[pb][tid] += first;
       }
       __syncthreads();
@@ -429,13 +494,13 @@
           for (int j = 0; j < IPT; ++j) r[j] = sk[j * RS_THREADS + tid];
 #pragma unroll
           for (int j = 0; j < IPT; ++j) {
-            const uint32_t dg = ((uint32_t)r[j] >> shift) & (CM_RADIX - 1);
+            const uint32_t dg = sort_digit<NB>((uint32_t)r[j], shift, idx_mask);
             out[ssc[dg] + (j * RS_THREADS + tid)] = r[j];
           }
         } else {
           for (uint32_t pos = tid; pos < prev_n; pos += RS_THREADS) {
             const unsigned long long r = sk[pos];
-            const uint32_t dg = ((uint32_t)r >> shift) & (CM_RADIX - 1);
+            const uint32_t dg = sort_digit<NB>((uint32_t)r, shift, idx_mask);
             out[ssc[dg] + pos] = r;
           }
         }
@@ -486,9 +551,13 @@
   }
   if (FUSED0) {
     __syncthreads();
-    for (uint32_t i = tid; i < 3u * CM_RADIX; i += RS_THREADS) {
-      const uint32_t c = (&sm.later[0][0])[i];
-      if (c && (i >> 8) + 1u < si.num_passes) atomicAdd(p.hist + CM_RADIX + i, c);
+    if (SEG) {
+      flush_later();
+    } else {
+      for (uint32_t i = tid; i < 3u * CM_RADIX; i += RS_THREADS) {
+        const uint32_t c = sm.later[i];
+        if (c && (i >> 8) + 1u < si.num_passes) atomicAdd(p.hist + CM_RADIX + i, c);
+      }
     }
   }
 }
@@ -535,22 +604,24 @@
 }
 
 namespace {
-template <typename KeyT, int IPT, bool FUSED0 = false, bool SEG = false>
+template <typename KeyT, int IPT, bool FUSED0 = false, bool SEG = false, int NB = CM_RADIX>
 struct PassLaunch {
+  using Smem = SortSmem<KeyT, IPT, NB, FUSED0 && SEG>;
+  static constexpr uint32_t SCANNERS = NB / RS_SCAN_DIGITS;
   static inline int ctas_per_sm = 0;
   static cudaError_t configure() {
-    cudaError_t e = cudaFuncSetAttribute(k_onesweep_pass<KeyT, IPT, FUSED0, SEG>, cudaFuncAttributeMaxDynamicSharedMemorySize,
-                                         (int)sizeof(SortSmem<KeyT, IPT>));
+    cudaError_t e = cudaFuncSetAttribute(k_onesweep_pass<KeyT, IPT, FUSED0, SEG, NB>, cudaFuncAttributeMaxDynamicSharedMemorySize,
+                                         (int)sizeof(Smem));
     if (e != cudaSuccess) return e;
-    return cudaOccupancyMaxActiveBlocksPerMultiprocessor(&ctas_per_sm, k_onesweep_pass<KeyT, IPT, FUSED0, SEG>, RS_THREADS,
-                                                         sizeof(SortSmem<KeyT, IPT>));
+    return cudaOccupancyMaxActiveBlocksPerMultiprocessor(&ctas_per_sm, k_onesweep_pass<KeyT, IPT, FUSED0, SEG, NB>, RS_THREADS,
+                                                         sizeof(Smem));
   }
   static cudaError_t launch(const VoxelParams& p, int pass, int sms, cudaStream_t stream) {
     const uint32_t tile = RS_THREADS * IPT;
     const uint32_t tiles = (p.max_points + tile - 1) / tile + (SEG ? p.n_frames : 0u);
     if (tiles == 0) return cudaSuccess;
-    const uint32_t workers = std::min<uint32_t>(tiles, (uint32_t)(sms * std::max(1, ctas_per_sm)) - RS_SCANNERS);
-    k_onesweep_pass<KeyT, IPT, FUSED0, SEG><<<workers + RS_SCANNERS, RS_THREADS, sizeof(SortSmem<KeyT, IPT>), stream>>>(p, pass);
+    const uint32_t workers = std::min<uint32_t>(tiles, (uint32_t)(sms * std::max(1, ctas_per_sm)) - SCANNERS);
+    k_onesweep_pass<KeyT, IPT, FUSED0, SEG, NB><<<workers + SCANNERS, RS_THREADS, sizeof(Smem), stream>>>(p, pass);
     return cudaGetLastError();
   }
 };
@@ -567,12 +638,18 @@
   if (e == cudaSuccess) e = PassLaunch<uint32_t, RS_IPT_SMALL, true>::configure();
   if (e == cudaSuccess) e = PassLaunch<uint32_t, SortCfg<uint32_t>::IPT, false, true>::configure();
   if (e == cudaSuccess) e = PassLaunch<uint32_t, RS_IPT_SMALL, false, true>::configure();
+  if (e == cudaSuccess) e = PassLaunch<uint32_t, SortCfg<uint32_t>::IPT, true, true>::configure();
+  if (e == cudaSuccess) e = PassLaunch<uint32_t, RS_IPT_SMALL, true, true>::configure();
+  if (e == cudaSuccess) e = PassLaunch<uint32_t, SortCfg<uint32_t>::IPT, false, true, CM_WIDE_BINS>::configure();
+  if (e == cudaSuccess) e = PassLaunch<uint32_t, RS_IPT_SMALL, false, true, CM_WIDE_BINS>::configure();
   if (e != cudaSuccess) return e;
   if (getenv("CM_DEBUG"))
-    fprintf(stderr, "[cm] sort pass CTAs per SM: %d / %d (32 / 64-bit keys), small tile %d / %d\n",
+    fprintf(stderr, "[cm] sort pass CTAs per SM: %d / %d (32 / 64-bit keys), small tile %d / %d, wide top digit %d / %d\n",
             PassLaunch<uint32_t, SortCfg<uint32_t>::IPT>::ctas_per_sm,
             PassLaunch<unsigned long long, SortCfg<unsigned long long>::IPT>::ctas_per_sm,
-            PassLaunch<uint32_t, RS_IPT_SMALL>::ctas_per_sm, PassLaunch<unsigned long long, RS_IPT_SMALL>::ctas_per_sm);
+            PassLaunch<uint32_t, RS_IPT_SMALL>::ctas_per_sm, PassLaunch<unsigned long long, RS_IPT_SMALL>::ctas_per_sm,
+            PassLaunch<uint32_t, SortCfg<uint32_t>::IPT, false, true, CM_WIDE_BINS>::ctas_per_sm,
+            PassLaunch<uint32_t, RS_IPT_SMALL, false, true, CM_WIDE_BINS>::ctas_per_sm);
   g_sort_configured = true;
   return cudaSuccess;
 }
@@ -582,6 +659,17 @@
   cudaGetDevice(&dev);
   cudaDeviceGetAttribute(&sms, cudaDevAttrMultiProcessorCount, dev);
   const bool small = sort_uses_small_tile(p.max_points);
+  if (p.fused_keys && p.box.seg_sort) {
+    constexpr int I = SortCfg<uint32_t>::IPT;
+    if (pass == 0)
+      return small ? PassLaunch<uint32_t, RS_IPT_SMALL, true, true>::launch(p, pass, sms, stream)
+                   : PassLaunch<uint32_t, I, true, true>::launch(p, pass, sms, stream);
+    if ((uint32_t)pass + 1u == p.box.n_pass && p.box.top_bins > CM_RADIX)
+      return small ? PassLaunch<uint32_t, RS_IPT_SMALL, false, true, CM_WIDE_BINS>::launch(p, pass, sms, stream)
+                   : PassLaunch<uint32_t, I, false, true, CM_WIDE_BINS>::launch(p, pass, sms, stream);
+    return small ? PassLaunch<uint32_t, RS_IPT_SMALL, false, true>::launch(p, pass, sms, stream)
+                 : PassLaunch<uint32_t, I, false, true>::launch(p, pass, sms, stream);
+  }
   if (p.fused_keys && pass == 0)
     return small ? PassLaunch<uint32_t, RS_IPT_SMALL, true>::launch(p, pass, sms, stream)
                  : PassLaunch<uint32_t, SortCfg<uint32_t>::IPT, true>::launch(p, pass, sms, stream);
diff --git a/cloud_merger_b200/csrc/cm_transform_crop.cu b/cloud_merger_b200/csrc/cm_transform_crop.cu
--- a/cloud_merger_b200/csrc/cm_transform_crop.cu
+++ b/cloud_merger_b200/csrc/cm_transform_crop.cu
@@ -372,7 +372,7 @@
     __syncthreads();
     if (tid < CM_RADIX) {
       const uint32_t c = s_hist[tid];
-      if (c) atomicAdd(p.hist + tid, c);
+      if (c) atomicAdd(p.hist + sg->frame * p.hist_frame_stride + tid, c);
     }
   }
   K1_TRACE(5);
diff --git a/cloud_merger_b200/csrc/cm_voxel.cu b/cloud_merger_b200/csrc/cm_voxel.cu
--- a/cloud_merger_b200/csrc/cm_voxel.cu
+++ b/cloud_merger_b200/csrc/cm_voxel.cu
@@ -209,7 +209,7 @@
   if (ts.rec) tile_scan_body(ts.rec, ts.n_tiles, ts.segs, ts.n_seg, p.n_frames, const_cast<uint32_t*>(p.frame_surv_start),
                              ts.seg_surv_start, s_scr);
   __syncthreads();
-  if (ts.rec && p.fused_keys) {
+  if (ts.rec && p.fused_keys && !p.box.seg_sort) {
     const unsigned long long T = p.sort_tile;
     for (uint32_t i = tid; i < ts.n_tiles; i += SCAN_THREADS) {
       const uint32_t c = ts.rec[i].count;
@@ -289,6 +289,7 @@
     bool seg = p.segmented == 2u;
     if (p.segmented == 1u) seg = !has_invalid && idx_bits <= 32u;
     if (seg) frame_bits = 0u;
+    const bool fused_seg = p.fused_keys && p.box.seg_sort;
     uint32_t width = p.key_bytes;
     if (p.dual_width) width = p.segmented == 1u ? (seg ? 4u : 8u) : (frame_bits + idx_bits <= 32u ? 4u : 8u);
     uint32_t total = frame_bits + idx_bits;
@@ -297,7 +298,7 @@
       total = width * 8u;
       idx_bits = total - frame_bits;
     }
-    uint32_t passes = (total + CM_RADIX_BITS - 1) / CM_RADIX_BITS;
+    uint32_t passes = fused_seg ? p.box.n_pass : (total + CM_RADIX_BITS - 1) / CM_RADIX_BITS;
     if (passes == 0) passes = 1;
     if (passes > p.max_passes) {
       atomicExch(&p.ctrl->error, (uint32_t)CM_DEV_E_KEY_RANGE);
@@ -312,10 +313,11 @@
     si.width = width;
     si.segmented = seg ? 1u : 0u;
     si.n_seg_tiles = 0;
+    si.seg_sort = (seg || fused_seg) ? 1u : 0u;
     s_si = si;
   }
   __syncthreads();
-  if (s_si.segmented) {
+  if (s_si.seg_sort) {
     const uint32_t T = p.sort_tile, F = p.n_frames;
     uint32_t carry = 0;
     for (uint32_t f0 = 0; f0 < F; f0 += SCAN_THREADS) {
@@ -341,7 +343,25 @@
         p.seg_tile[t0 + t] = st;
       }
     }
-    const uint32_t M = s_si.n_keys;
+    if (p.fused_keys) {
+      for (uint32_t i = tid; i < ts.n_tiles; i += SCAN_THREADS) {
+        const TileRec r = ts.rec[i];
+        if (!r.count) continue;
+        const uint32_t fs = p.frame_surv_start[r.frame];
+        const uint32_t t = (r.dense0 - fs + T - 1u) / T;
+        if (fs + (unsigned long long)t * T < (unsigned long long)r.dense0 + r.count) p.first_k1[p.seg_frame_tile0[r.frame] + t] = i;
+      }
+      for (uint32_t f = warp; f < F; f += SCAN_THREADS / 32) {
+        uint32_t* h = p.seg_hist + (size_t)f * (CM_SEG_PASSES * CM_RADIX) + lane * 8u;
+        uint32_t c[8], sum = 0;
+#pragma unroll
+        for (int k = 0; k < 8; ++k) { c[k] = h[k]; sum += c[k]; }
+        uint32_t run = p.frame_surv_start[f] + warp_incl_scan_u32(sum) - sum;
+#pragma unroll
+        for (int k = 0; k < 8; ++k) { h[k] = run; run += c[k]; }
+      }
+    }
+    const uint32_t M = s_si.segmented ? s_si.n_keys : 0u;
     auto frame_from = [&](uint32_t i, uint32_t lo) {
       uint32_t hi = F - 1u;
       while (lo < hi) {
@@ -486,15 +506,18 @@
   }
 }
 
-__global__ void __launch_bounds__(CM_RADIX) k_seg_base(const VoxelParams p) {
-  __shared__ uint32_t s_scan[12];
+template <int NB>
+__global__ void __launch_bounds__(NB) k_seg_base(const VoxelParams p) {
+  __shared__ uint32_t s_scan[NB / 32 + 4];
   const SortInfo si = *p.info;
-  if (!si.segmented || blockIdx.y >= si.num_passes) return;
+  constexpr uint32_t first_pass = NB > CM_RADIX ? 1u : 0u;
+  if (!si.seg_sort || blockIdx.y < first_pass || blockIdx.y >= si.num_passes) return;
   const uint32_t f = blockIdx.x, tid = threadIdx.x;
   uint32_t* h = p.seg_hist + ((size_t)f * CM_SEG_PASSES + blockIdx.y) * CM_RADIX;
+  const uint32_t nb = (NB > CM_RADIX && blockIdx.y + 1u == si.num_passes) ? p.box.top_bins : CM_RADIX;
   uint32_t tot;
-  const uint32_t ex = block_excl_scan_256(h[tid], s_scan, &tot);
-  h[tid] = p.frame_surv_start[f] + ex;
+  const uint32_t ex = block_excl_scan<NB>(tid < nb ? h[tid] : 0u, s_scan, &tot);
+  if (tid < nb) h[tid] = p.frame_surv_start[f] + ex;
 }
 
 __global__ void __launch_bounds__(VX_THREADS) k_seg_keys64(const uint2* __restrict__ rec, unsigned long long* __restrict__ keys,
@@ -1080,7 +1103,10 @@
 
 cudaError_t launch_seg_base(const VoxelParams& p, cudaStream_t stream) {
   if (p.n_frames == 0) return cudaSuccess;
-  k_seg_base<<<dim3(p.n_frames, CM_SEG_PASSES), CM_RADIX, 0, stream>>>(p);
+  if (p.fused_keys && p.box.seg_sort)
+    k_seg_base<CM_WIDE_BINS><<<dim3(p.n_frames, CM_SEG_PASSES), CM_WIDE_BINS, 0, stream>>>(p);
+  else
+    k_seg_base<CM_RADIX><<<dim3(p.n_frames, CM_SEG_PASSES), CM_RADIX, 0, stream>>>(p);
   return cudaGetLastError();
 }
 
```
